# agsiddhant/PBML_Mantle_Convection

Measured on AMD Instinct MI355X. Metric: training samples/sec (2-D 506x506 Stokes fields), higher is better.
Workload: dtype f16+bf16; 1 GPU; CFG-3: symmetric U-Net (levels 5, c_h 16, k 5, repeats 3, reflect) + L1 data loss + divergence + Stokes momentum residual, 506x506, per-GPU batch 32, Adam, HIP-graph replay; global_batch=32, parallelism=dp1

## Files before the change

### include/mantle_hip.h

```cpp
#ifndef MANTLE_HIP_H
#define MANTLE_HIP_H

#include <stddef.h>
#include <stdint.h>

#ifdef __cplusplus
extern "C" {
#endif

#define MC_OK 0
#define MC_EINVAL (-1)
#define MC_EUNSUPPORTED (-2)
#define MC_EWORKSPACE (-3)

enum { MC_F32 = 0, MC_BF16 = 1, MC_MIX16 = 2 };
enum { MC_PAD_ZEROS = 0, MC_PAD_REPLICATE = 1, MC_PAD_REFLECT = 2 };
enum { MC_ACT_NONE = 0, MC_ACT_GELU = 1, MC_ACT_RELU = 2, MC_ACT_SILU = 3, MC_ACT_TANH = 4,
       MC_ACT_SELU = 5, MC_ACT_ELU = 6 };
enum { MC_POST_NONE = 0,
       MC_POST_ACT = 1,
       MC_POST_GN_ACT = 2   };
enum { MC_GSRC_NONE = 0,
       MC_GSRC_PLAIN = 1,
       MC_GSRC_PADFOLD = 2,
       MC_GSRC_PADFOLD_POOL = 3,
       MC_GSRC_PLAIN_POOL = 4   };

typedef struct {
  int32_t n;
  int32_t h, w;
  int32_t c_in0;
  int32_t c_in1;
  int32_t c_out;
  int32_t k;
  int32_t pad;
  int32_t pad_mode;
  int32_t dtype;
  int32_t sym_h;
  int32_t c_out_split;
  int32_t out_f32;
  int32_t sym_v;
  int32_t sym_hv;
} mc_conv_desc;

typedef struct {
  const void* ptr;
  int32_t kind;
  int32_t pad;
  int32_t pad_mode;
  int32_t pool;
  int32_t hs, ws;
  int32_t c8_total;
  int32_t cb_off;
} mc_grad_src;

typedef struct {
  const float* coef0;
  const float* coef1;
  int32_t act0, act1;
} mc_conv_prologue;

typedef struct {
  const void* y;
  const float* coef;
  int32_t act;
  int32_t pad;
  int32_t pad_mode;
  int32_t hs, ws;
  float* partials;
  int32_t part_stride;
  int32_t y_f16;
} mc_conv_epilogue;

int mc_version(void);
const char* mc_strerror(int code);

int mc_pack_nchw(const float* x, int32_t n, int32_t c, int32_t src_c, int32_t h, int32_t w, int32_t pad_w,
                 int32_t pad_mode, const float* chan_scale, int32_t dtype, void* out, void* stream);
int mc_unpack_nchw(const void* x, int32_t n, int32_t c, int32_t h, int32_t w, int32_t crop_w,
                   const float* mean_nc, int32_t dtype, float* out, void* stream);
int mc_pack_grad_nchw(const float* g, int32_t n, int32_t c, int32_t h, int32_t w, int32_t crop_w,
                      const float* mean_nc, int32_t dtype, void* out, void* stream);
int mc_sum_hw(const float* x, int32_t nc, int32_t hw, float scale, float* out, void* stream);

size_t mc_packed_weight_bytes(const mc_conv_desc* d, int32_t dgrad);
int mc_pack_weights(const mc_conv_desc* d, const float* w_unique, int32_t dgrad, void* packed,
                    void* stream);
const char* mc_conv_kernel_name(const mc_conv_desc* d);
int32_t mc_conv_tiles(const mc_conv_desc* d);
int mc_conv2d(const mc_conv_desc* d, const void* x0, const void* x1, const void* packed_w,
              const float* bias, void* y0, void* y1, float* stat_partials, void* stream);
int mc_conv2d_fused(const mc_conv_desc* d, const void* x0, const void* x1, const mc_conv_prologue* pro,
                    const void* packed_w, const float* bias, void* y0, void* y1, float* stat_partials,
                    const mc_conv_epilogue* epi, void* stream);
size_t mc_wgrad_partial_bytes(const mc_conv_desc* d);
size_t mc_conv_bank_read_extent(const mc_conv_desc* d);
int mc_conv2d_wgrad(const mc_conv_desc* d, const void* x0, const void* x1, const void* dy,
                    void* partials, void* stream);
int mc_conv2d_wgrad_finalize(const mc_conv_desc* d, const void* partials, float* dw_unique,
                             float* dbias, void* stream);
int mc_conv2d_wgrad_fused(const mc_conv_desc* d, const void* x0, const void* x1, const mc_conv_prologue* pro,
                          const void* dy, void* partials, void* stream);
int mc_pack_weights_batched(const mc_conv_desc* descs, const float* const* w_unique, const int32_t* dgrad,
                            void* const* packed, int32_t n, void* stream);
int mc_conv2d_wgrad_finalize_batched(const mc_conv_desc* descs, const void* const* partials, float* const* dw_unique,
                                     float* const* dbias, int32_t n, void* stream);

int mc_fold_padded(void* buf, int32_t n, int32_t c, int32_t hs, int32_t ws, int32_t pad, int32_t pad_mode,
                   int32_t dtype, void* stream);
int mc_fold_padded2(void* buf0, int32_t c0, void* buf1, int32_t c1, int32_t n, int32_t hs, int32_t ws, int32_t pad, int32_t pad_mode,
                    int32_t dtype, void* stream);
int32_t mc_fold_blocks(int32_t hs, int32_t ws, int32_t pad, int32_t pad_mode);
int mc_fold_padded_dz(void* buf, int32_t n, int32_t c, int32_t hs, int32_t ws, int32_t pad, int32_t pad_mode,
                      int32_t dtype, const void* y, const float* coef, int32_t act, float* partials,
                      int32_t part_stride_blocks, int32_t part_first_block, void* stream);

int mc_gn_partials(const void* y, int32_t n, int32_t c, int32_t h, int32_t w, int32_t dtype, int32_t tiles, float* part,
                   void* stream);
int mc_gn_finalize(const float* stat_partials, int32_t n, int32_t tiles, int32_t c, int32_t groups,
                   int32_t hw, float eps, float* stats_ng2, float* chan_mean, void* stream);
int mc_gn_finalize_coef(const float* stat_partials, int32_t n, int32_t tiles, int32_t c, int32_t groups, int32_t hw,
                        float eps, const float* gamma, const float* beta, float* stats_ng2, float* coef4, void* stream);

int mc_gn_act_fwd(const void* y, int32_t n, int32_t c, int32_t h, int32_t w, int32_t groups,
                  const float* stats_ng2, const float* gamma, const float* beta, int32_t post,
                  int32_t act, int32_t pool, int32_t dtype, void* a, void* pooled, void* stream);
int mc_gn_act_fwd_small(const void* y, const float* stat_partials, int32_t tiles, int32_t n, int32_t c, int32_t h, int32_t w,
                        int32_t groups, float eps, const float* gamma, const float* beta, int32_t act, int32_t pool,
                        int32_t dtype, float* stats_ng2, void* a, void* pooled, void* stream);
int32_t mc_gn_bwd_blocks(int32_t h, int32_t w);
int mc_gn_act_bwd_reduce(const void* y, int32_t n, int32_t c, int32_t h, int32_t w, int32_t groups,
                         const float* stats_ng2, const float* gamma, const float* beta, int32_t post,
                         int32_t act, int32_t dtype, const mc_grad_src* g0, const mc_grad_src* g1,
                         float* partials, void* stream);
int mc_gn_act_bwd_finalize(const float* partials, int32_t n, int32_t blocks, int32_t c, int32_t groups,
                           int32_t hw, const float* gamma, float* m12_ng2, float* dgamma, float* dbeta,
                           void* stream);
int mc_gn_act_bwd_finalize_n(const float* partials, int32_t n, int32_t blocks, int32_t c, int32_t groups, int32_t hw,
                             const float* gamma, float* m12_ng2, float* chan_sums, void* stream);
int mc_gn_act_bwd_apply(const void* y, int32_t n, int32_t c, int32_t h, int32_t w, int32_t groups,
                        const float* stats_ng2, const float* m12_ng2, const float* gamma,
                        const float* beta, int32_t post, int32_t act, int32_t dtype,
                        const mc_grad_src* g0, const mc_grad_src* g1, void* dy, void* stream);
int mc_gn_act_bwd_small(const void* y, int32_t n, int32_t c, int32_t h, int32_t w, int32_t groups, const float* stats_ng2,
                        const float* gamma, const float* beta, int32_t act, int32_t dtype, const mc_grad_src* g0,
                        const mc_grad_src* g1, void* dy, float* chan_sums, void* stream);
int mc_gn_param_grads_batched(const float* const* chan_sums, const int32_t* n, const int32_t* c, float* const* dgamma,
                              float* const* dbeta, int32_t jobs, void* stream);
int mc_gn_bwd_apply_dz(const mc_grad_src* dz, const void* y, int32_t n, int32_t c, int32_t h, int32_t w, int32_t groups,
                       const float* coef, const float* m12_ng2, int32_t dtype, void* dy, void* stream);
int mc_concat_cb8(const void* const* srcs, const int32_t* src_c, int32_t n_src, int32_t n, int32_t h, int32_t w,
                  int32_t dtype, void* out, void* stream);
int mc_cat_grad_gather(const mc_grad_src* g, int32_t c_total, int32_t c_off, int32_t c, int32_t n, int32_t h, int32_t w,
                       int32_t dtype, void* out, void* stream);
int mc_gsrc_sum(const mc_grad_src* g0, const mc_grad_src* g1, int32_t n, int32_t c, int32_t h, int32_t w,
                int32_t dtype, void* out, void* stream);

int mc_rect_copy(const void* src, int32_t hs, int32_t ws, int32_t sy, int32_t sx, void* dst, int32_t hd, int32_t wd,
                 int32_t dy, int32_t dx, int32_t rh, int32_t rw, int32_t n, int32_t c, int32_t accumulate, int32_t dtype,
                 void* stream);

typedef struct {
  int32_t n;
  int32_t h, w;
  int32_t c_in, c_out;
  int32_t k;
  int32_t bc_x, bc_y;
  int32_t dtype;
  int32_t sym_h;
} mc_learned_desc;

int32_t mc_learned_validate(const mc_learned_desc* d);
size_t mc_learned_bank_bytes(const mc_learned_desc* d, int32_t dgrad);
size_t mc_learned_wgrad_workspace_bytes(const mc_learned_desc* d);
int mc_learned_pack_banks_batched(const mc_learned_desc* descs, const float* const* w_unique, void* const* fwd_banks,
                                  void* const* dgrad_banks, int32_t n, void* stream);
int mc_learned_frame_fwd(const mc_learned_desc* d, const void* x, const void* fwd_bank, const float* bias, void* y,
                         void* stream);
int mc_learned_frame_dgrad(const mc_learned_desc* d, const void* dy, const void* dgrad_bank, void* dx, void* stream);
int mc_learned_frame_wgrad(const mc_learned_desc* d, const void* x, const void* dy, void* workspace,
                           float* const* dw_unique, float* dbias, void* stream);

int mc_avgpool_fwd(const void* x, int32_t n, int32_t c, int32_t h, int32_t w, int32_t f, int32_t dtype,
                   void* out, void* stream);
int mc_bicubic_fwd(const void* x, int32_t n, int32_t c, int32_t hi, int32_t wi, int32_t ho, int32_t wo,
// ... 95 lines not shown
```

### pbml_mantle_convection_amd/_lib.py

```python
import ctypes as C
import os

import torch

_HERE = os.path.dirname(os.path.abspath(__file__))
LIB_PATH = os.environ.get("MANTLE_LIB", os.path.join(_HERE, "libmantle_hip.so"))

MC_F32, MC_BF16, MC_MIX16 = 0, 1, 2
PAD_MODES = {"zeros": 0, "constant": 0, "replicate": 1, "reflect": 2}
ACTS = {"none": 0, "gelu": 1, "relu": 2, "silu": 3, "tanh": 4, "selu": 5, "elu": 6}
POST_NONE, POST_ACT, POST_GN_ACT = 0, 1, 2
GSRC_NONE, GSRC_PLAIN, GSRC_PADFOLD, GSRC_PADFOLD_POOL, GSRC_PLAIN_POOL = 0, 1, 2, 3, 4
LOSS_SLOTS = 16
LOSS_TYPES = {"mae": 0, "mass": 1, "curl": 2}


class ConvDesc(C.Structure):
    _fields_ = [(n, C.c_int32) for n in ("n", "h", "w", "c_in0", "c_in1", "c_out", "k", "pad", "pad_mode",
                                          "dtype", "sym_h", "c_out_split", "out_f32", "sym_v", "sym_hv")]


class LearnedDesc(C.Structure):
    _fields_ = [(n, C.c_int32) for n in ("n", "h", "w", "c_in", "c_out", "k", "bc_x", "bc_y", "dtype", "sym_h")]


LEARNED_FRAME_BANKS = ("conv_bottom_left", "conv_bottom", "conv_bottom_right", "conv_left", "conv_right", "conv_top_left",
                       "conv_top", "conv_top_right")


class GradSrc(C.Structure):
    _fields_ = [("ptr", C.c_void_p), ("kind", C.c_int32), ("pad", C.c_int32), ("pad_mode", C.c_int32),
                ("pool", C.c_int32), ("hs", C.c_int32), ("ws", C.c_int32), ("c8_total", C.c_int32), ("cb_off", C.c_int32)]


class ConvPrologue(C.Structure):
    _fields_ = [("coef0", C.c_void_p), ("coef1", C.c_void_p), ("act0", C.c_int32), ("act1", C.c_int32)]


class ConvEpilogue(C.Structure):
    _fields_ = [("y", C.c_void_p), ("coef", C.c_void_p), ("act", C.c_int32), ("pad", C.c_int32), ("pad_mode", C.c_int32),
                ("hs", C.c_int32), ("ws", C.c_int32), ("partials", C.c_void_p), ("part_stride", C.c_int32),
                ("y_f16", C.c_int32)]


class LossDesc(C.Structure):
    _fields_ = [("n", C.c_int32), ("h", C.c_int32), ("w", C.c_int32), ("p_pred", C.c_int32),
                ("loss_type", C.c_int32), ("loss_scale", C.c_int32), ("loss_derivative", C.c_int32),
                ("l2", C.c_int32), ("lambda_mom", C.c_float), ("inv_h", C.c_float), ("ra", C.c_float),
                ("t_grad", C.c_int32)]


_vp, _i32, _i64, _f32, _sz = C.c_void_p, C.c_int32, C.c_int64, C.c_float, C.c_size_t
_CD, _GS, _LD = C.POINTER(ConvDesc), C.POINTER(GradSrc), C.POINTER(LossDesc)
_CP, _CE = C.POINTER(ConvPrologue), C.POINTER(ConvEpilogue)
_LN = C.POINTER(LearnedDesc)

SIGNATURES = {
    "mc_version": (C.c_int, []),
    "mc_strerror": (C.c_char_p, [C.c_int]),
    "mc_pack_nchw": (C.c_int, [_vp, _i32, _i32, _i32, _i32, _i32, _i32, _i32, _vp, _i32, _vp, _vp]),
    "mc_unpack_nchw": (C.c_int, [_vp, _i32, _i32, _i32, _i32, _i32, _vp, _i32, _vp, _vp]),
    "mc_pack_grad_nchw": (C.c_int, [_vp, _i32, _i32, _i32, _i32, _i32, _vp, _i32, _vp, _vp]),
    "mc_sum_hw": (C.c_int, [_vp, _i32, _i32, _f32, _vp, _vp]),
    "mc_packed_weight_bytes": (_sz, [_CD, _i32]),
    "mc_conv_bank_read_extent": (_sz, [_CD]),
    "mc_pack_weights": (C.c_int, [_CD, _vp, _i32, _vp, _vp]),
    "mc_conv_tiles": (_i32, [_CD]),
    "mc_conv_kernel_name": (C.c_char_p, [_CD]),
    "mc_conv2d": (C.c_int, [_CD, _vp, _vp, _vp, _vp, _vp, _vp, _vp, _vp]),
    "mc_conv2d_fused": (C.c_int, [_CD, _vp, _vp, _CP, _vp, _vp, _vp, _vp, _vp, _CE, _vp]),
    "mc_conv2d_wgrad_fused": (C.c_int, [_CD, _vp, _vp, _CP, _vp, _vp, _vp]),
    "mc_gn_finalize_coef": (C.c_int, [_vp, _i32, _i32, _i32, _i32, _i32, _f32, _vp, _vp, _vp, _vp, _vp]),
    "mc_fold_blocks": (_i32, [_i32, _i32, _i32, _i32]),
    "mc_fold_padded_dz": (C.c_int, [_vp, _i32, _i32, _i32, _i32, _i32, _i32, _i32, _vp, _vp, _i32, _vp, _i32, _i32, _vp]),
    "mc_gn_bwd_apply_dz": (C.c_int, [_GS, _vp, _i32, _i32, _i32, _i32, _i32, _vp, _vp, _i32, _vp, _vp]),
    "mc_bicubic_fwd_act": (C.c_int, [_vp, _vp, _i32, _i32, _i32, _i32, _i32, _i32, _i32, _vp, _vp, _vp, _vp, _i32, _vp,
                                     _vp]),
    "mc_wgrad_partial_bytes": (_sz, [_CD]),
    "mc_conv2d_wgrad": (C.c_int, [_CD, _vp, _vp, _vp, _vp, _vp]),
    "mc_conv2d_wgrad_finalize": (C.c_int, [_CD, _vp, _vp, _vp, _vp]),
    "mc_pack_weights_batched": (C.c_int, [_CD, _vp, _vp, _vp, _i32, _vp]),
    "mc_conv2d_wgrad_finalize_batched": (C.c_int, [_CD, _vp, _vp, _vp, _i32, _vp]),
    "mc_fold_padded": (C.c_int, [_vp, _i32, _i32, _i32, _i32, _i32, _i32, _i32, _vp]),
    "mc_fold_padded2": (C.c_int, [_vp, _i32, _vp, _i32, _i32, _i32, _i32, _i32, _i32, _i32, _vp]),
    "mc_gn_partials": (C.c_int, [_vp, _i32, _i32, _i32, _i32, _i32, _i32, _vp, _vp]),
    "mc_gn_finalize": (C.c_int, [_vp, _i32, _i32, _i32, _i32, _i32, _f32, _vp, _vp, _vp]),
    "mc_gn_act_fwd": (C.c_int, [_vp, _i32, _i32, _i32, _i32, _i32, _vp, _vp, _vp, _i32, _i32, _i32, _i32, _vp,
                                _vp, _vp]),
    "mc_gn_bwd_blocks": (_i32, [_i32, _i32]),
    "mc_gn_act_bwd_reduce": (C.c_int, [_vp, _i32, _i32, _i32, _i32, _i32, _vp, _vp, _vp, _i32, _i32, _i32, _GS,
                                       _GS, _vp, _vp]),
    "mc_gn_act_bwd_finalize": (C.c_int, [_vp, _i32, _i32, _i32, _i32, _i32, _vp, _vp, _vp, _vp, _vp]),
    "mc_gn_act_bwd_finalize_n": (C.c_int, [_vp, _i32, _i32, _i32, _i32, _i32, _vp, _vp, _vp, _vp]),
    "mc_gn_act_bwd_apply": (C.c_int, [_vp, _i32, _i32, _i32, _i32, _i32, _vp, _vp, _vp, _vp, _i32, _i32, _i32,
                                      _GS, _GS, _vp, _vp]),
    "mc_gn_act_fwd_small": (C.c_int, [_vp, _vp, _i32, _i32, _i32, _i32, _i32, _i32, _f32, _vp, _vp, _i32, _i32, _i32, _vp, _vp, _vp,
                                      _vp]),
    "mc_gn_act_bwd_small": (C.c_int, [_vp, _i32, _i32, _i32, _i32, _i32, _vp, _vp, _vp, _i32, _i32, _GS, _GS, _vp, _vp, _vp]),
    "mc_gn_param_grads_batched": (C.c_int, [_vp, _vp, _vp, _vp, _vp, _i32, _vp]),
    "mc_avgpool_fwd": (C.c_int, [_vp, _i32, _i32, _i32, _i32, _i32, _i32, _vp, _vp]),
    "mc_rect_copy": (C.c_int, [_vp, _i32, _i32, _i32, _i32, _vp, _i32, _i32, _i32, _i32, _i32, _i32, _i32, _i32, _i32, _i32,
                               _vp]),
    "mc_learned_validate": (_i32, [_LN]),
    "mc_learned_bank_bytes": (_sz, [_LN, _i32]),
    "mc_learned_wgrad_workspace_bytes": (_sz, [_LN]),
    "mc_learned_pack_banks_batched": (C.c_int, [_LN, _vp, _vp, _vp, _i32, _vp]),
    "mc_learned_frame_fwd": (C.c_int, [_LN, _vp, _vp, _vp, _vp, _vp]),
    "mc_learned_frame_dgrad": (C.c_int, [_LN, _vp, _vp, _vp, _vp]),
    "mc_learned_frame_wgrad": (C.c_int, [_LN, _vp, _vp, _vp, _vp, _vp, _vp]),
    "mc_concat_cb8": (C.c_int, [_vp, _vp, _i32, _i32, _i32, _i32, _i32, _vp, _vp]),
    "mc_gsrc_sum": (C.c_int, [_GS, _GS, _i32, _i32, _i32, _i32, _i32, _vp, _vp]),
    "mc_cat_grad_gather": (C.c_int, [_GS, _i32, _i32, _i32, _i32, _i32, _i32, _i32, _vp, _vp]),
    "mc_bicubic_fwd": (C.c_int, [_vp, _i32, _i32, _i32, _i32, _i32, _i32, _vp, _vp, _vp, _vp, _i32, _vp, _vp]),
    "mc_bicubic_bwd": (C.c_int, [_GS, _i32, _i32, _i32, _i32, _i32, _i32, _vp, _vp, _vp, _vp, _vp, _vp, _i32,
                                 _vp, _vp]),
    "mc_bicubic_bwd_walk": (C.c_int, [_GS, _i32, _i32, _i32, _i32, _i32, _i32, _vp, _vp, _vp, _vp, _vp, _vp, _vp, _i32, _i32, _vp, _vp]),
    "mc_bicubic_bwd_taps": (C.c_int, [_GS, _i32, _i32, _i32, _i32, _i32, _i32, _vp, _vp, _vp, _vp, _vp, _vp, _i32, _i32, _i32,
                                      _vp, _vp]),
    "mc_bicubic_bwd_separable": (C.c_int, [_GS, _i32, _i32, _i32, _i32, _i32, _i32, _vp, _vp, _vp, _vp, _vp, _vp, _i32,
                                           _vp, _vp, _vp]),
    "mc_curl_head_fwd": (C.c_int, [_vp, _vp, _i32, _i32, _i32, _i64, _f32, _f32, _f32, _vp, _vp, _vp, _vp]),
    "mc_curl_head_bwd": (C.c_int, [_vp, _vp, _vp, _vp, _i32, _i32, _i32, _f32, _f32, _f32, _vp, _vp, _i64, _i64,
                                   _vp, _vp]),
    "mc_curl_valid_fwd": (C.c_int, [_vp, _i32, _i32, _i32, _i64, _f32, _vp, _vp, _vp]),
    "mc_curl_valid_bwd": (C.c_int, [_vp, _vp, _i32, _i32, _i32, _f32, _vp, _i64, _vp]),
    "mc_assemble_adtime_batch": (C.c_int, [_vp, _vp, _vp, _vp, _vp, _vp, _vp, _vp, _i32, _i32, _i32, _i32, _i32, _vp, _vp,
                                           _vp, _vp, _vp]),
    "mc_assemble_newad_batch": (C.c_int, [_vp, _vp, _vp, _vp, _vp, _vp, _vp, _vp, _i32, _i32, _i32, _i32, _i32, _vp, _vp, _vp, _vp, _vp]),
    "mc_ts_build_input": (C.c_int, [_vp, _vp, _vp, _vp, _vp, _vp, _i32, _i32, _i32, _vp, _vp]),
    "mc_ts_build_input_unet": (C.c_int, [_vp, _vp, _vp, _vp, _vp, _vp, _vp, _vp, _vp, _i32, _i32, _i32, _vp, _vp]),
    "mc_roll_forward_update": (C.c_int, [_vp, _i32, _vp, _vp, _vp, _i64, _vp, _i32, _i32, _i32, _i32, _vp]),
    "mc_ts_wall_bc": (C.c_int, [_vp, _i32, _i32, _i32, _vp, _vp]),
    "mc_adnet_step": (C.c_int, [_vp, _vp, _i64, _vp, _vp, _vp, _vp, _vp, _vp, _i32, _i32, _i32, _f32, _i32, _vp, _vp, _vp,
                                _vp]),
    "mc_loss_minmax": (C.c_int, [_vp, _i32, _i32, _i32, _i32, _vp, _vp]),
    "mc_loss_fwd_bwd": (C.c_int, [_LD, _vp, _vp, _vp, _vp, _i64, _i64, _vp, _vp, _vp, _vp, _vp, _vp, _vp, _vp]),
    "mc_loss_fused": (C.c_int, [_LD, _vp, _vp, _vp, _vp, _i64, _i64, _vp, _i32, _i32, _vp, _i32, _vp, _vp, _vp, _vp, _vp, _vp, _vp, _vp,
                                _vp, _vp, _i64, _i64, _vp, _vp]),
    "mc_loss_fused_blocks": (_i32, [_i32, _i32, _i32]),
    "mc_partial_sums_finalize": (C.c_int, [_vp, _i32, _i32, _i32, _f32, _vp, _vp]),
    "mc_momentum_residual": (C.c_int, [_LD, _vp, _vp, _vp, _vp, _i64, _i64, _vp, _vp, _vp, _vp, _vp, _vp, _vp, _vp]),
    "mc_momentum_adjoint": (C.c_int, [_LD, _vp, _i64, _i64, _vp, _vp, _vp, _vp, _vp, _vp, _vp, _vp, _vp, _vp]),
    "mc_loss_finalize": (C.c_int, [_LD, _vp, _vp, _vp]),
    "mc_adam_step_flat": (C.c_int, [_vp, _vp, _vp, _vp, _i64, _vp, _f32, _f32, _f32, _f32, _f32, _vp, _vp]),
}

VALUE_RETURNING = {"mc_version", "mc_strerror", "mc_conv_kernel_name", "mc_packed_weight_bytes", "mc_conv_bank_read_extent", "mc_conv_tiles",
                   "mc_wgrad_partial_bytes", "mc_gn_bwd_blocks",
                   "mc_learned_validate", "mc_learned_bank_bytes", "mc_learned_wgrad_workspace_bytes", "mc_fold_blocks", "mc_loss_fused_blocks"}

_lib = None


def load():
# ... 50 lines not shown
```

### pbml_mantle_convection_amd/build_ext.py

```python
import os
import subprocess
import sys

HERE = os.path.dirname(os.path.abspath(__file__))
CSRC = os.path.join(HERE, "csrc")
LIB = os.path.join(HERE, "libmantle_hip.so")
SOURCES = ["elementwise.hip", "conv_api.hip", "conv_f32.hip", "conv_bf16.hip", "conv_rr_bf16.hip", "conv_learned.hip", "loss.hip", "optim.hip"]
HEADERS = ["common.h", "conv_common.h", "conv_rr.h", os.path.join("..", "..", "include", "mantle_hip.h")]
FLAGS = ["-O3", "--offload-arch=gfx950", "-fPIC", "-std=c++17", "-Wall", "-Wno-unused-function",
         "-ffp-contract=off"]


EXTRA_FLAGS = {"conv_rr_bf16.hip": ["-fno-slp-vectorize"]}


def _stale(target, deps):
    if not os.path.exists(target):
        return True
    t = os.path.getmtime(target)
    return any(os.path.getmtime(d) > t for d in deps)


def build(force=False, verbose=True):
    hipcc = os.environ.get("HIPCC", "/opt/rocm/bin/hipcc")
    hdrs = [os.path.join(CSRC, h) for h in HEADERS]
    objdir = os.path.join(HERE, "build")
    os.makedirs(objdir, exist_ok=True)
    objs = []
    procs = []
    for src in SOURCES:
        s = os.path.join(CSRC, src)
        o = os.path.join(objdir, src.replace(".hip", ".o"))
        objs.append(o)
        if force or _stale(o, [s] + hdrs):
            cmd = [hipcc, *FLAGS, *EXTRA_FLAGS.get(src, []), "-c", s, "-o", o]
            if verbose:
                print(" ".join(cmd), flush=True)
            procs.append((src, subprocess.Popen(cmd)))
    for src, p in procs:
        if p.wait() != 0:
            raise RuntimeError(f"hipcc failed on {src}")
    if force or procs or _stale(LIB, objs):
        cmd = [hipcc, "--offload-arch=gfx950", "-shared", "-fPIC", *objs, "-o", LIB]
        if verbose:
            print(" ".join(cmd), flush=True)
        subprocess.check_call(cmd)
    return LIB


if __name__ == "__main__":
    build(force="--force" in sys.argv)
    print(LIB)
```

### pbml_mantle_convection_amd/csrc/common.h

```cpp
#pragma once
#include <hip/hip_runtime.h>
#include <stdint.h>
#include "../../include/mantle_hip.h"

typedef uint16_t bf16_t;

#define MC_CHECK_LAUNCH()                                 \
  do {                                                    \
    hipError_t e__ = hipGetLastError();                   \
    if (e__ != hipSuccess) return (int)e__;               \
  } while (0)

static inline int cdiv(int a, int b) { return (a + b - 1) / b; }

__device__ __forceinline__ float bf2f(bf16_t v) { return __uint_as_float(((uint32_t)v) << 16); }
__device__ __forceinline__ bf16_t f2bf(float f) {
  __bf16 b = (__bf16)f;
  return __builtin_bit_cast(bf16_t, b);
}
typedef float mc_f32x2 __attribute__((ext_vector_type(2)));
typedef __bf16 mc_bf16x2 __attribute__((ext_vector_type(2)));
__device__ __forceinline__ uint32_t pk_bf16(float a, float b) {
  return __builtin_bit_cast(uint32_t, __builtin_convertvector((mc_f32x2){a, b}, mc_bf16x2));
}
// ... 177 lines not shown
}
template <bool FAST>
__device__ __forceinline__ void act_bwd8(const float (&v)[8], const float (&sc)[8], const float (&sh)[8], int act, float (&o)[8]) {
  if (FAST && act == MC_ACT_GELU) {
#pragma unroll
    for (int j = 0; j < 8; j += 2) {
      f32x2 z = pk_fma((f32x2){v[j], v[j + 1]}, (f32x2){sc[j], sc[j + 1]}, (f32x2){sh[j], sh[j + 1]});
      f32x2 r = gelu_grad_poly2(z);
      o[j] = r.x; o[j + 1] = r.y;
    }
  } else {
#pragma unroll
    for (int j = 0; j < 8; ++j) o[j] = act_bwd(v[j] * sc[j] + sh[j], act);
  }
}
template <typename T> struct FastMath { static constexpr bool value = false; };
template <> struct FastMath<bf16_t> { static constexpr bool value = true; };
template <> struct FastMath<f16_t> { static constexpr bool value = true; };
__host__ __device__ inline bool mc_is16(int dtype) { return dtype == MC_BF16 || dtype == MC_MIX16; }

__device__ __forceinline__ void load_coef8(const float* __restrict__ coef4, int n, int CP, int cb, float (&sc)[8], float (&sh)[8]) {
  if (coef4) {
    const float4* p = reinterpret_cast<const float4*>(coef4) + (size_t)n * CP + cb * 8;
#pragma unroll
    for (int j = 0; j < 8; ++j) { const float4 v = p[j]; sc[j] = v.x; sh[j] = v.y; }
  } else {
#pragma unroll
    for (int j = 0; j < 8; ++j) { sc[j] = 1.f; sh[j] = 0.f; }
  }
}
__device__ __forceinline__ uint4 xform_bf16x8(uint4 a, const float (&sc)[8], const float (&sh)[8], int act) {
  float v[8];
  v[0] = __uint_as_float(a.x << 16); v[1] = __uint_as_float(a.x & 0xffff0000u);
  v[2] = __uint_as_float(a.y << 16); v[3] = __uint_as_float(a.y & 0xffff0000u);
  v[4] = __uint_as_float(a.z << 16); v[5] = __uint_as_float(a.z & 0xffff0000u);
  v[6] = __uint_as_float(a.w << 16); v[7] = __uint_as_float(a.w & 0xffff0000u);
  act_fwd8<true>(v, sc, sh, act, v);
  uint4 o;
  o.x = pk_bf16(v[0], v[1]);
  o.y = pk_bf16(v[2], v[3]);
  o.z = pk_bf16(v[4], v[5]);
  o.w = pk_bf16(v[6], v[7]);
  return o;
}

__device__ __forceinline__ uint4 xform_f16x8(uint4 a, const float (&sc)[8], const float (&sh)[8], int act) {
  float v[8];
  V8<f16_t>::ld(reinterpret_cast<const f16_t*>(&a), v);
  act_fwd8<true>(v, sc, sh, act, v);
  return make_uint4(pk_f16(v[0], v[1]), pk_f16(v[2], v[3]), pk_f16(v[4], v[5]), pk_f16(v[6], v[7]));
}
__device__ __forceinline__ uint4 f16x8_to_bf16x8(uint4 a) {
  const mc_f32x2 x = unpk_f16(a.x), y = unpk_f16(a.y), z = unpk_f16(a.z), w = unpk_f16(a.w);
  return make_uint4(pk_bf16(x.x, x.y), pk_bf16(y.x, y.y), pk_bf16(z.x, z.y), pk_bf16(w.x, w.y));
}

__device__ __forceinline__ float wave_sum(float v) {
#pragma unroll
  for (int o = 32; o > 0; o >>= 1) v += __shfl_xor(v, o, 64);
  return v;
}
__device__ __forceinline__ double wave_sum_d(double v) {
#pragma unroll
  for (int o = 32; o > 0; o >>= 1) v += __shfl_xor(v, o, 64);
  return v;
}

__device__ __forceinline__ float wave_sum16(const float (&s)[16], int lane, int& idx) {
  float t[8], u[4], v[2], w;
  const bool b5 = lane & 32, b4 = lane & 16, b3 = lane & 8, b2 = lane & 4;
#pragma unroll
  for (int k = 0; k < 8; ++k) t[k] = (b5 ? s[8 + k] : s[k]) + __shfl_xor(b5 ? s[k] : s[8 + k], 32, 64);
#pragma unroll
  for (int k = 0; k < 4; ++k) u[k] = (b4 ? t[4 + k] : t[k]) + __shfl_xor(b4 ? t[k] : t[4 + k], 16, 64);
#pragma unroll
  for (int k = 0; k < 2; ++k) v[k] = (b3 ? u[2 + k] : u[k]) + __shfl_xor(b3 ? u[k] : u[2 + k], 8, 64);
  w = (b2 ? v[1] : v[0]) + __shfl_xor(b2 ? v[0] : v[1], 4, 64);
  w += __shfl_xor(w, 2, 64);
  w += __shfl_xor(w, 1, 64);
  idx = (b5 ? 8 : 0) + (b4 ? 4 : 0) + (b3 ? 2 : 0) + (b2 ? 1 : 0);
  return w;
}

__device__ __forceinline__ int fold_candidates(int i, int n, int p, int mode, int (&out)[6]) {
  int cnt = 0;
  out[cnt++] = i + p;
  if (mode == MC_PAD_REFLECT) {
    if (i >= 1 && i <= p) out[cnt++] = p - i;
    int j = 2 * (n - 1) - i;
    if (j >= n && j < n + p) out[cnt++] = j + p;
  } else if (mode == MC_PAD_REPLICATE) {
    if (i == 0) for (int q = 0; q < p && cnt < 6; ++q) out[cnt++] = q;
    if (i == n - 1) for (int q = 0; q < p && cnt < 6; ++q) out[cnt++] = n + p + q;
  }
  return cnt;
}

template <typename T, int KIND = -1>
__device__ __forceinline__ void grad_fetch_add(const mc_grad_src& g, int n, int cb, int y, int x, int C8,
                                               float (&acc)[8]) {
  const int kind = KIND >= 0 ? KIND : g.kind;
  if (kind == MC_GSRC_NONE || (KIND < 0 && g.ptr == nullptr)) return;
  const T* base = reinterpret_cast<const T*>(g.ptr);
  if (KIND < 0 && g.c8_total > 0) { C8 = g.c8_total; cb += g.cb_off; }
  float v[8];
  if (kind == MC_GSRC_PLAIN) {
    V8<T>::ld(base + cb8_index(n, cb, y, x, C8, g.hs, g.ws), v);
#pragma unroll
    for (int j = 0; j < 8; ++j) acc[j] += v[j];
    return;
  }
  float scale = 1.0f;
  int yy = y, xx = x;
  if (kind == MC_GSRC_PADFOLD_POOL || kind == MC_GSRC_PLAIN_POOL) {
    if (g.pool == 2) { yy = y >> 1; xx = x >> 1; } else { yy = y / g.pool; xx = x / g.pool; }
    if (yy >= g.hs || xx >= g.ws) return;
    scale = 1.0f / (float)(g.pool * g.pool);
  }
  const int pad = kind == MC_GSRC_PLAIN_POOL ? 0 : g.pad;
  V8<T>::ld(base + cb8_index(n, cb, yy + pad, xx + pad, C8, g.hs + 2 * pad, g.ws + 2 * pad), v);
#pragma unroll
  for (int j = 0; j < 8; ++j) acc[j] += scale * v[j];
}
```

### pbml_mantle_convection_amd/csrc/conv_api.hip

```cpp
#include "conv_rr.h"

int mc_conv2d_f32(const ConvGeom& g, const void* x0, const void* x1, const void* bank, const float* bias, void* y0,
                  void* y1, float* part, const ConvFuse& fz, int fuse, hipStream_t s);
int mc_wgrad_f32(const ConvGeom& g, const void* x0, const void* x1, const void* dy, void* part, const ConvFuse& fz, int fuse,
                 hipStream_t s);
int mc_bf16_tile(const mc_conv_desc* d, int* th, int* tw);
size_t mc_bf16_bank_bytes(const ConvGeom& g, int dgrad);
int mc_conv2d_bf16(const ConvGeom& g, const void* x0, const void* x1, const void* bank, const float* bias, void* y0,
                   void* y1, float* part, const ConvFuse& fz, int fuse, hipStream_t s);
int mc_wgrad_bf16(const ConvGeom& g, const void* x0, const void* x1, const void* dy, void* part, const ConvFuse& fz, int fuse,
                  hipStream_t s);
const char* mc_bf16_kernel_name(const ConvGeom& g);
void mc_bf16_bank_dims(const ConvGeom& g, int dgrad, int& chunks, int& steps, int& ntiles);
bool mc_rr_applies(int dtype, int cout, int wo, bool full_pad);
size_t mc_rr_bank_bytes(const ConvGeom& g, int dgrad);
int mc_conv2d_rr(const ConvGeom& g, const void* x0, const void* x1, const void* bank, const float* bias, void* y0, void* y1,
                 float* part, const ConvFuse& fz, int fuse, hipStream_t s);
const char* mc_rr_kernel_name(const ConvGeom& g, int fuse);

namespace {

bool rr_desc(const mc_conv_desc* d) {
  return mc_rr_applies(d->dtype, d->c_out, d->w + 2 * d->pad - d->k + 1, d->pad == d->k - 1);
}

int geom_for(const mc_conv_desc* d, ConvGeom& g) {
  if (!d) return MC_EINVAL;
  int th = 16, tw = 16;
  if (mc_is16(d->dtype)) {
    if (rr_desc(d)) { th = RR_R; tw = RR_TW; }
    else {
      int rc = mc_bf16_tile(d, &th, &tw);
      if (rc) return rc;
    }
  } else if (d->dtype != MC_F32) {
    return MC_EUNSUPPORTED;
  }
  return conv_geom(d, th, tw, g);
}
int stat_slots(const mc_conv_desc* d, const ConvGeom& g) { return rr_desc(d) ? g.tiles * RR_STRIPS : g.tiles; }

struct PkJob {
  int K, Cout, CBin, CB0, Cin0, Cin1, Cin, U, nh, nv, nq, CBout, CinP, CoutP;
  int dgrad, steps, ntiles, bf16, f16, rr, first_block;
  unsigned total;
  const float* w;
  void* out;
};
constexpr int PK_MAX = 24;
struct PkTable { int n; PkJob j[PK_MAX]; };

__global__ void k_pack_batched(PkTable t) {
  int ji = 0;
#pragma unroll 1
  for (int k = 1; k < t.n; ++k) if ((int)blockIdx.x >= t.j[k].first_block) ji = k;
  const PkJob& job = t.j[ji];
  const int nblk = (ji + 1 < t.n ? t.j[ji + 1].first_block : (int)gridDim.x) - job.first_block;
  for (size_t i = (size_t)(blockIdx.x - job.first_block) * blockDim.x + threadIdx.x; i < job.total; i += (size_t)nblk * blockDim.x) {
    if (job.rr || job.bf16) {
      const float v = job.rr ? rr_pack_value(job, job.w, i, job.dgrad, job.ntiles)
                             : pack_value_bf16(job, job.w, i, job.dgrad, job.steps, job.ntiles);
      reinterpret_cast<bf16_t*>(job.out)[i] = job.f16 ? __builtin_bit_cast(bf16_t, (_Float16)v) : f2bf(v);
    } else {
      reinterpret_cast<float*>(job.out)[i] = pack_value_f32(job, job.w, i, job.dgrad);
    }
  }
}

struct WfJob {
  int K, U, nh, nv, nq, Cin, Cin0, CB0, CinP, CoutP, Cout, G, first_block;
  const float* part;
  float* dw;
  float* db;
};
constexpr int WF_MAX = 32;
struct WfTable { int n; WfJob j[WF_MAX]; };

constexpr int WF_WAVES = 16;
__device__ __forceinline__ void wgrad_finalize_block(const WfJob& g, int lblock) {
  const int K = g.K, KK = K * K;
  const int nch = wg_chunks(g.CinP);
  const size_t slab = wg_slab_floats(g.CoutP, g.CinP, KK);
  const size_t nW = (size_t)KK * nch * g.U * 16;
  const size_t total = nW + g.Cout;
  const int e = threadIdx.x & 63, w = threadIdx.x >> 6, NWV = (int)blockDim.x >> 6;
  const size_t i = (size_t)lblock * 64 + e;
  __shared__ float red[WF_WAVES][64];
  float s = 0.f;
  long dst = -1;
  if (i < total) {
    size_t o1, ox[3] = {0, 0, 0};
    int nx = 0;
    bool live = true;
    if (i < nW) {
// ... 105 lines not shown
  if (geom_for(d, g)) return "unsupported";
  if (rr_desc(d)) return mc_rr_kernel_name(g, 0);
  if (mc_is16(g.dtype)) return mc_bf16_kernel_name(g);
  return g.K == 5 ? "k_conv_direct_f32<5>" : "k_conv_direct_f32<3>";
}

int32_t mc_conv_tiles(const mc_conv_desc* d) {
  ConvGeom g;
  if (geom_for(d, g)) return -1;
  return stat_slots(d, g);
}

static bool act_ok(int a) { return a >= MC_ACT_NONE && a <= MC_ACT_ELU; }

static int fill_prologue(const mc_conv_prologue* pro, ConvFuse& fz, int& rc) {
  rc = MC_OK;
  if (!pro) return 0;
  if (!act_ok(pro->act0) || !act_ok(pro->act1)) { rc = MC_EINVAL; return 0; }
  fz.coef0 = pro->coef0; fz.coef1 = pro->coef1; fz.act0 = pro->act0; fz.act1 = pro->act1;
  return (pro->coef0 || pro->coef1 || pro->act0 != MC_ACT_NONE || pro->act1 != MC_ACT_NONE) ? 1 : 0;
}

int mc_conv2d_fused(const mc_conv_desc* d, const void* x0, const void* x1, const mc_conv_prologue* pro,
                    const void* packed_w, const float* bias, void* y0, void* y1, float* stat_partials,
                    const mc_conv_epilogue* epi, void* stream) {
  ConvGeom g;
  int rc = geom_for(d, g);
  if (rc) return rc;
  if (!x0 || !packed_w || !y0 || (g.Cin1 > 0 && !x1) || (g.split8 > 0 && !y1)) return MC_EINVAL;
  ConvFuse fz = conv_fuse_none();
  int fuse = fill_prologue(pro, fz, rc);
  if (rc) return rc;
  if (epi) {
    if (fuse) return MC_EUNSUPPORTED;
    if (!epi->y || !epi->partials || !act_ok(epi->act) || epi->pad < 0 || epi->hs <= 0 || epi->ws <= 0) return MC_EINVAL;
    if (epi->pad_mode < MC_PAD_ZEROS || epi->pad_mode > MC_PAD_REFLECT) return MC_EINVAL;
    if (g.split8 > 0 || stat_partials || g.out_f32) return MC_EUNSUPPORTED;
    if (g.Ho != epi->hs + 2 * epi->pad || g.Wo != epi->ws + 2 * epi->pad) return MC_EINVAL;
    fz.ey = epi->y; fz.ecoef = epi->coef; fz.epart = epi->partials; fz.eact = epi->act; fz.epad = epi->pad;
    fz.ezero = epi->pad_mode == MC_PAD_ZEROS || epi->pad == 0; fz.ehs = epi->hs; fz.ews = epi->ws;
    if (epi->y_f16 && g.dtype != MC_BF16) return MC_EINVAL;
    fz.ey16 = epi->y_f16 ? 1 : 0;
    if (epi->part_stride < stat_slots(d, g)) return MC_EINVAL;
    fz.estride = epi->part_stride;
    fuse = 2;
  }
  if (rr_desc(d)) return mc_conv2d_rr(g, x0, x1, packed_w, bias, y0, y1, stat_partials, fz, fuse, (hipStream_t)stream);
  if (mc_is16(g.dtype)) return mc_conv2d_bf16(g, x0, x1, packed_w, bias, y0, y1, stat_partials, fz, fuse, (hipStream_t)stream);
  return mc_conv2d_f32(g, x0, x1, packed_w, bias, y0, y1, stat_partials, fz, fuse, (hipStream_t)stream);
}

int mc_conv2d(const mc_conv_desc* d, const void* x0, const void* x1, const void* packed_w, const float* bias, void* y0,
              void* y1, float* stat_partials, void* stream) {
  return mc_conv2d_fused(d, x0, x1, nullptr, packed_w, bias, y0, y1, stat_partials, nullptr, stream);
}

size_t mc_conv_bank_read_extent(const mc_conv_desc* d) {
  ConvGeom g;
  if (geom_for(d, g)) return 0;
  const int KK = g.K * g.K;
  if (rr_desc(d)) {
    const size_t nfrag = g.K == 5 ? RR<5>::NFRAG : RR<3>::NFRAG;
    const size_t chunks = (g.CBin + 1) / 2, groups = (g.Cout + 15) / 16;
    return (((chunks - 1) * groups + (groups - 1)) * nfrag * 64 + (nfrag * 64 - 1)) * 16 + 16;
  }
  if (mc_is16(g.dtype)) {
    int chunks, steps, ntiles;
    mc_bf16_bank_dims(g, 0, chunks, steps, ntiles);
    const size_t last = ((size_t)(chunks - 1) * steps + (steps - 1)) * ntiles + (ntiles - 1);
    return (last * 64 + 63) * 16 + 16;
  }
  const int ncog = (g.CoutP + 15) / 16, co0 = 16 * (ncog - 1);
  const int comax = g.CoutP - 1 - co0;
  const size_t last = (((size_t)(g.CBin - 1) * KK + (KK - 1)) * 8 + 7) * g.CoutP + co0 + (comax >= 15 ? 15 : comax);
  return (last + 1) * sizeof(float);
}

size_t mc_wgrad_partial_bytes(const mc_conv_desc* d) {
  ConvGeom g;
  if (geom_for(d, g)) return 0;
  return (size_t)g.wgrad_G * wg_slab_floats(g.CoutP, g.CinP, g.K * g.K) * sizeof(float);
}

int mc_conv2d_wgrad_fused(const mc_conv_desc* d, const void* x0, const void* x1, const mc_conv_prologue* pro,
                          const void* dy, void* partials, void* stream) {
  ConvGeom g;
  int rc = geom_for(d, g);
  if (rc) return rc;
  if (!x0 || !dy || !partials || (g.Cin1 > 0 && !x1)) return MC_EINVAL;
  ConvFuse fz = conv_fuse_none();
  const int fuse = fill_prologue(pro, fz, rc);
  if (rc) return rc;
  if (mc_is16(g.dtype)) return mc_wgrad_bf16(g, x0, x1, dy, partials, fz, fuse, (hipStream_t)stream);
  return mc_wgrad_f32(g, x0, x1, dy, partials, fz, fuse, (hipStream_t)stream);
}

int mc_conv2d_wgrad(const mc_conv_desc* d, const void* x0, const void* x1, const void* dy, void* partials,
                    void* stream) {
  return mc_conv2d_wgrad_fused(d, x0, x1, nullptr, dy, partials, stream);
}

int mc_conv2d_wgrad_finalize_batched(const mc_conv_desc* descs, const void* const* partials, float* const* dw,
                                     float* const* db, int32_t n, void* stream) {
  if (!descs || !partials || !dw || !db || n <= 0) return MC_EINVAL;
  for (int pass = 0; pass < 2; ++pass) {
    WfTable t;
    t.n = 0;
    int blocks = 0;
    auto flush = [&]() {
      if (t.n == 0) return;
      hipLaunchKernelGGL(k_wgrad_finalize, dim3(blocks), dim3(pass == 0 ? 64 * WF_WAVES : 256), 0, (hipStream_t)stream, t);
      t.n = 0; blocks = 0;
    };
    for (int k = 0; k < n; ++k) {
      WfJob j;
      int b = 0;
      int rc = wf_fill(&descs[k], partials[k], dw[k], db[k], j, b);
      if (rc) return rc;
      if ((j.G >= 128) != (pass == 0)) continue;
      j.first_block = blocks;
      t.j[t.n++] = j;
      blocks += b;
      if (t.n == WF_MAX) flush();
    }
    flush();
    MC_CHECK_LAUNCH();
  }
  return MC_OK;
}

int mc_conv2d_wgrad_finalize(const mc_conv_desc* d, const void* partials, float* dw_unique, float* dbias,
                             void* stream) {
  return mc_conv2d_wgrad_finalize_batched(d, &partials, &dw_unique, &dbias, 1, stream);
}

int mc_pack_weights_batched(const mc_conv_desc* descs, const float* const* w_unique, const int32_t* dgrad,
                            void* const* packed, int32_t n, void* stream) {
  if (!descs || !w_unique || !dgrad || !packed || n <= 0) return MC_EINVAL;
  for (int base = 0; base < n; base += PK_MAX) {
    PkTable t;
    t.n = n - base < PK_MAX ? n - base : PK_MAX;
    int blocks = 0;
    for (int k = 0; k < t.n; ++k) {
      ConvGeom g;
      int rc = geom_for(&descs[base + k], g);
      if (rc) return rc;
      if (!w_unique[base + k] || !packed[base + k]) return MC_EINVAL;
      PkJob& j = t.j[k];
      j.K = g.K; j.Cout = g.Cout; j.CBin = g.CBin; j.CB0 = g.CB0; j.Cin0 = g.Cin0; j.Cin1 = g.Cin1; j.Cin = g.Cin; j.U = g.U;
      j.nh = g.nh; j.nv = g.nv; j.nq = g.nq;
      j.CBout = g.CBout; j.CinP = g.CinP; j.CoutP = g.CoutP; j.dgrad = dgrad[base + k]; j.bf16 = mc_is16(g.dtype);
      j.f16 = (g.dtype == MC_MIX16 && !j.dgrad) ? 1 : 0;
      j.rr = bank_is_rr(g, j.dgrad);
      size_t total;
      if (j.rr) {
        j.steps = 0;
        j.ntiles = ((j.dgrad ? g.CinP : g.Cout) + 15) / 16;
        total = mc_rr_bank_bytes(g, j.dgrad) / 2;
      } else if (j.bf16) {
        int chunks;
        mc_bf16_bank_dims(g, j.dgrad, chunks, j.steps, j.ntiles);
        total = (size_t)chunks * j.steps * j.ntiles * 64 * 8;
      } else {
        j.steps = 0; j.ntiles = 0;
        total = (size_t)(j.dgrad ? g.CBout : g.CBin) * g.K * g.K * 8 * (j.dgrad ? g.CinP : g.CoutP);
      }
      j.total = (unsigned)total;
      j.w = w_unique[base + k];
      j.out = packed[base + k];
      j.first_block = blocks;
      int b = (int)((total + 256 * 8 - 1) / (256 * 8));
      blocks += b < 1 ? 1 : b;
    }
    hipLaunchKernelGGL(k_pack_batched, dim3(blocks), dim3(256), 0, (hipStream_t)stream, t);
    MC_CHECK_LAUNCH();
  }
  return MC_OK;
// ... 12 lines not shown
```

### pbml_mantle_convection_amd/csrc/conv_bf16.hip

```cpp
#include "conv_common.h"
#include <type_traits>

using bf16x8 = __attribute__((ext_vector_type(8))) short;
using f16x8 = __attribute__((ext_vector_type(8))) _Float16;
using f32x4 = __attribute__((ext_vector_type(4))) float;
typedef unsigned int v4u __attribute__((ext_vector_type(4)));

namespace {

constexpr int CHUNK_CB = 2;

template <int K> struct KSteps { static constexpr int pairs = K * K * CHUNK_CB; static constexpr int steps = (pairs + 3) / 4; };

struct Bf16Cfg { int th, tw, nt, mt; };

__host__ __device__ inline int pick_nt(int n_tiles) { return (n_tiles % 4 == 0) ? 4 : ((n_tiles % 2 == 0) ? 2 : 1); }


template <bool H16> __device__ __forceinline__ f32x4 mfma16(bf16x8 a, bf16x8 b, f32x4 c) {
  if constexpr (H16) return __builtin_amdgcn_mfma_f32_16x16x32_f16(__builtin_bit_cast(f16x8, a), __builtin_bit_cast(f16x8, b), c, 0, 0, 0);
  else return __builtin_amdgcn_mfma_f32_16x16x32_bf16(a, b, c, 0, 0, 0);
}

template <int K, int TH, int TW, int NT, int MT, bool OUT_F32 = false, int FUSE = 0, bool H16 = false, int WN = 1>
__global__ __launch_bounds__(64 * (TH * (TW / 16) / MT) * WN, 2) void k_conv_mfma_bf16(
    ConvGeom g, const bf16_t* __restrict__ x0, const bf16_t* __restrict__ x1, const bf16_t* __restrict__ bank,
    const float* __restrict__ bias, bf16_t* __restrict__ y0, bf16_t* __restrict__ y1, float* __restrict__ part,
    int n_groups, ConvFuse fz) {
  constexpr int TIH = TH + K - 1, TIW = TW + K - 1;
  constexpr int PLANE = (TIH * TIW + 15) / 16 * 16;
  constexpr int STEPS = KSteps<K>::steps;
  constexpr int MTILES_X = TW / 16;
  constexpr int WAVES = TH * MTILES_X / MT * WN, NTHR = 64 * WAVES;
  constexpr int NTW = NT / WN;
  static_assert(TH * MTILES_X * WN == WAVES * MT && NTW * WN == NT && (WAVES == 4 || WAVES == 8), "tile / wave decomposition mismatch");
  constexpr int IN_SLOTS = CHUNK_CB * PLANE;
  constexpr bool WGLOBAL = NT > 1;
  constexpr int W_SLOTS = WGLOBAL ? 0 : STEPS * NT * 64;
  static_assert(!OUT_F32 || NT == 1, "f32 output is for the single-N-tile configuration");
  constexpr int IN_ELEMS = CHUNK_CB * TIH * TIW;
  constexpr int IN_ITERS = (IN_ELEMS + NTHR - 1) / NTHR;
  constexpr int W_ITERS = WGLOBAL ? 1 : (W_SLOTS + NTHR - 1) / NTHR;
  __shared__ uint4 lds[IN_SLOTS + (WGLOBAL ? 1 : W_SLOTS)];
  __shared__ float red[WAVES][NT * 16 * 2];
  uint4* in_s = lds;
  uint4* w_s = lds + IN_SLOTS;

  const int grp = blockIdx.y;
  const int bid = xcd_remap(blockIdx.x, gridDim.x);
  const int lane = threadIdx.x & 63, wave = __builtin_amdgcn_readfirstlane(threadIdx.x >> 6);
  const int m = lane & 15, gq = lane >> 4;
  const int ntile0 = grp * NT;
  const int wm = wave / WN, nt_w0 = (wave % WN) * NTW;
  const int ntiles_total = gridDim.y * NT;
  const int chunks = (g.CBin + CHUNK_CB - 1) / CHUNK_CB;
  const int items = g.N * g.tiles;
  const int my_items = (items - bid + (int)gridDim.x - 1) / (int)gridDim.x;
  const int total_stages = my_items * chunks;

  constexpr int PER_CB = (TIH * TIW + NTHR - 1) / NTHR;
  static_assert(IN_ITERS <= CHUNK_CB * PER_CB, "");
  v4u rin[CHUNK_CB][PER_CB];
  float psc[CHUNK_CB][8], psh[CHUNK_CB][8];
  int pact[CHUNK_CB] = {-1, -1};
  unsigned okm = 0xffffffffu;
  int s_rc[PER_CB];
  unsigned s_off[PER_CB];
  int s_lds[PER_CB];
#pragma unroll
  for (int it = 0; it < PER_CB; ++it) {
    int i = threadIdx.x + it * NTHR;
    bool live = i < TIH * TIW;
    if (!live) i = TIH * TIW - 1;
    int r = i / TIW, c = i - r * TIW;
    s_rc[it] = (live ? 0 : (1 << 31)) | (r << 15) | c;
    s_off[it] = (unsigned)(r * g.W + c) * 16u;
    s_lds[it] = live ? r * TIW + c : -1;
  }
  auto prefetch = [&](int t) {
    const int jitem = t / chunks, ck = t - jitem * chunks;
    const int wi = bid + jitem * (int)gridDim.x;
    const int n = wi / g.tiles, tile = wi - n * g.tiles;
    const int ty0 = (tile / g.tiles_x) * TH, tx0 = (tile % g.tiles_x) * TW;
// ... 243 lines not shown
          const size_t off = (size_t)(i / MTILES_X) * row_bytes + (size_t)(i % MTILES_X) * 16 * 8 * 2;
          float yf[4];
          if constexpr (H16) {
            const f32x2 ya = unpk_f16(yv[i].x), yb = unpk_f16(yv[i].y);
            yf[0] = ya.x; yf[1] = ya.y; yf[2] = yb.x; yf[3] = yb.y;
          } else {
            yf[0] = __uint_as_float(yv[i].x << 16); yf[1] = __uint_as_float(yv[i].x & 0xffff0000u);
            yf[2] = __uint_as_float(yv[i].y << 16); yf[3] = __uint_as_float(yv[i].y & 0xffff0000u);
          }
          float o[4];
#pragma unroll
          for (int h = 0; h < 2; ++h) {
            const f32x2 yy = (f32x2){yf[2 * h], yf[2 * h + 1]};
            const f32x2 z = pk_fma(yy, (f32x2){csc[2 * h], csc[2 * h + 1]}, (f32x2){csh[2 * h], csh[2 * h + 1]});
            f32x2 gp;
            if (fz.eact == MC_ACT_GELU) gp = gelu_grad_poly2(z);
            else gp = (f32x2){act_bwd(z.x, fz.eact), act_bwd(z.y, fz.eact)};
            const f32x2 da = (f32x2){acc[i][tt][2 * h], acc[i][tt][2 * h + 1]};
            const f32x2 dz = da * gp;
            const f32x2 yh = (yy - (f32x2){cme[2 * h], cme[2 * h + 1]}) * (f32x2){crs[2 * h], crs[2 * h + 1]};
            if (fin[i]) { s1[tt][h] += dz; s2[tt][h] = pk_fma(dz, yh, s2[tt][h]); }
            o[2 * h] = fin[i] ? dz.x : da.x; o[2 * h + 1] = fin[i] ? dz.y : da.y;
          }
          if (inb && cobok[tt]) {
            uint2 pk;
            pk.x = (uint32_t)f2bf(o[0]) | ((uint32_t)f2bf(o[1]) << 16);
            pk.y = (uint32_t)f2bf(o[2]) | ((uint32_t)f2bf(o[3]) << 16);
            *reinterpret_cast<uint2*>(dst0[tt] + off) = pk;
          }
        }
      }
    };
    if constexpr (FUSE == 2) emit_dz();
    else { if (ty0 + TH <= g.Ho && tx0 + TW <= g.Wo) emit(std::true_type{}); else emit(std::false_type{}); }
    STAMP(5);
    if (FUSE == 2) part = fz.epart;
    if (part) {
#pragma unroll
      for (int tt = 0; tt < NTW; ++tt) {
        float q8[8] = {s1[tt][0].x, s2[tt][0].x, s1[tt][0].y, s2[tt][0].y, s1[tt][1].x, s2[tt][1].x, s1[tt][1].y, s2[tt][1].y};
        const bool b3 = m & 8, b2 = m & 4, b1 = m & 2;
        float q4[4], q2[2], q1;
#pragma unroll
        for (int k = 0; k < 4; ++k) q4[k] = (b3 ? q8[4 + k] : q8[k]) + __shfl_xor(b3 ? q8[k] : q8[4 + k], 8, 64);
#pragma unroll
        for (int k = 0; k < 2; ++k) q2[k] = (b2 ? q4[2 + k] : q4[k]) + __shfl_xor(b2 ? q4[k] : q4[2 + k], 4, 64);
        q1 = (b1 ? q2[1] : q2[0]) + __shfl_xor(b1 ? q2[0] : q2[1], 2, 64);
        q1 += __shfl_xor(q1, 1, 64);
        if ((m & 1) == 0) red[wave][((nt_w0 + tt) * 16 + gq * 4) * 2 + (m >> 1)] = q1;
      }
      __syncthreads();
      if (threadIdx.x < NT * 32) {
        int co = ntile0 * 16 + (threadIdx.x >> 1);
        if (co < g.CoutP) {
          float r = 0.f;
#pragma unroll
          for (int wv = 0; wv < WAVES / WN; ++wv) r += red[wv * WN + (int)(threadIdx.x >> 5) / NTW][threadIdx.x];
          part[(((size_t)n * (FUSE == 2 ? fz.estride : g.tiles) + tile) * g.CoutP + co) * 2 + (threadIdx.x & 1)] = r;
        }
      }
    }
    STAMP(6);
  }
#ifdef MC_EXP_STAMPS
  if (blockIdx.x == 777 && blockIdx.y == 0 && threadIdx.x == 0)
    printf("stamps tiles %d: wait1 %lld commit %lld wait2 %lld pfetch %lld kloop %lld epi %lld stats %lld\n", my_items, st_acc[0], st_acc[1], st_acc[2], st_acc[3], st_acc[4], st_acc[5], st_acc[6]);
#endif
}

typedef short v4s __attribute__((ext_vector_type(4)));
typedef __attribute__((address_space(3))) v4s lds_v4s;

__device__ __forceinline__ bf16x8 tr_frag(const short* base_lo) {
  v4s lo = __builtin_amdgcn_ds_read_tr16_b64_v4i16((lds_v4s*)base_lo);
  v4s hi = __builtin_amdgcn_ds_read_tr16_b64_v4i16((lds_v4s*)(base_lo + 32));
  return (bf16x8){lo[0], lo[1], lo[2], lo[3], hi[0], hi[1], hi[2], hi[3]};
}

constexpr int WTH = 16, WTW = 32;

template <int K, int NTW, bool PRO = false, bool XH = false>
__global__ __launch_bounds__(256, NTW == 1 ? 3 : 2) void k_wgrad_mfma_bf16(ConvGeom g, const bf16_t* __restrict__ x0,
                                                            const bf16_t* __restrict__ x1, const bf16_t* __restrict__ dy,
                                                            float* __restrict__ part, int tiles_x, int tiles, ConvFuse fz) {
  constexpr int NS = 4;
  constexpr int TPW = (K * K + NS) / NS;
  constexpr int KK = K * K;
  constexpr int TIH = WTH + K - 1, TIW = WTW + K - 1;
  constexpr int XRS = (TIW + 11) / 16 * 16 + 4;
  constexpr int DRS = WTW + 4;
  constexpr int XPS = (TIH * XRS + 15) / 16 * 16 + 8;
  constexpr int DPS = WTH * DRS + 8;
  static_assert(XRS >= TIW && XRS >= 3 * 8 + 12 && XRS % 16 == 4 && DRS % 16 == 4 && XPS % 16 == 8 && DPS % 16 == 8,
                "register-shift LDS layout");
  constexpr int NACC = TPW * NTW;
  constexpr int X_ITERS = (TIH * TIW + 255) / 256;
  constexpr int D_ELEMS = NTW * 2 * WTH * WTW, D_ITERS = D_ELEMS / 256;
  static_assert(D_ELEMS % 256 == 0, "dy tile must divide evenly over the threads");
  __shared__ uint4 smem[2 * XPS + NTW * 2 * DPS];
  uint4* const xs = smem;
  uint4* const ds = smem + 2 * XPS;
  const int chunk = blockIdx.y, cog = blockIdx.z;
  const int bid = xcd_remap(blockIdx.x, gridDim.x);
  const int lane = threadIdx.x & 63, tg = __builtin_amdgcn_readfirstlane(threadIdx.x >> 6);
  const int q = (lane & 15) >> 2, p = lane & 3, gq = lane >> 4;
  const int lane_x = ((p >> 1) * XPS + gq * XRS + q) * 8 + (p & 1) * 4;
  const int lane_d = ((p >> 1) * DPS + gq * DRS + q) * 8 + (p & 1) * 4;
  const short* xs_s = reinterpret_cast<const short*>(xs);
  const short* ds_s = reinterpret_cast<const short*>(ds);
  const bool do_bias = tg == NS - 1 && chunk == 0;
  const bf16x8 ones = (bf16x8){0x3F80, 0x3F80, 0x3F80, 0x3F80, 0x3F80, 0x3F80, 0x3F80, 0x3F80};
  const ptrdiff_t x1_delta = x1 ? reinterpret_cast<const char*>(x1) - reinterpret_cast<const char*>(x0) : (ptrdiff_t)0;

  int x_rc[X_ITERS];
  unsigned x_off[X_ITERS];
#pragma unroll
  for (int it = 0; it < X_ITERS; ++it) {
    int i = threadIdx.x + it * 256;
    bool live = i < TIH * TIW;
    if (!live) i = TIH * TIW - 1;
    int r = i / TIW, c = i - r * TIW;
    x_rc[it] = (live ? 0 : (1 << 31)) | (r << 15) | c;
    x_off[it] = (unsigned)(r * g.W + c) * 16u;
  }
  static_assert(WTW == 32 && WTH == 16, "dy staging decode");
  const int d_r0 = threadIdx.x >> 5, d_c0 = threadIdx.x & 31;
  const unsigned d_off0 = (unsigned)(d_r0 * g.Wo + d_c0) * 16u;
  const int d_lds0 = d_r0 * DRS + d_c0;
  const bool co_full = (cog * NTW + NTW) * 2 <= g.CBout;
  const char* xbase[2];
  bool xok[2];
  int xC8[2];
#pragma unroll
  for (int cb = 0; cb < 2; ++cb) {
    int gcb = chunk * 2 + cb;
    xok[cb] = gcb < g.CBin;
    int gcc = min(gcb, g.CBin - 1);
    bool second = gcc >= g.CB0;
    xC8[cb] = second ? g.CB1 : g.CB0;
    xbase[cb] = reinterpret_cast<const char*>(x0) + (second ? x1_delta : (ptrdiff_t)0) +
                cb8_index(0, second ? gcc - g.CB0 : gcc, 0, 0, xC8[cb], g.H, g.W) * sizeof(bf16_t);
  }

  uint4 rx[2][X_ITERS], rd[D_ITERS];
  float psc[2][8], psh[2][8];
  int pact[2] = {-1, -1};
  unsigned okm = 0xffffffffu;
  auto prefetch = [&](int wi_fwd) __attribute__((always_inline)) {
    const int wi = wi_fwd;
    const int n = wi / tiles, tile = wi - n * tiles;
    const int ty0 = (tile / tiles_x) * WTH, tx0 = (tile % tiles_x) * WTW;
    const bool interior = (ty0 - g.pad >= 0) && (ty0 - g.pad + TIH <= g.H) && (tx0 - g.pad >= 0) && (tx0 - g.pad + TIW <= g.W);
    const char* bpn[2] = {xbase[0] + (size_t)n * xC8[0] * g.H * g.W * 16, xbase[1] + (size_t)n * xC8[1] * g.H * g.W * 16};
    if constexpr (PRO) {
#pragma unroll
      for (int cb = 0; cb < 2; ++cb) {
        const int gcb = min(chunk * 2 + cb, g.CBin - 1);
        const bool second = gcb >= g.CB0;
        const float* ct = second ? fz.coef1 : fz.coef0;
        const int a = second ? fz.act1 : fz.act0;
        pact[cb] = (xok[cb] && (ct != nullptr || a != MC_ACT_NONE)) ? a : -1;
        if (pact[cb] >= 0) load_coef8(ct, n, xC8[cb] * 8, second ? gcb - g.CB0 : gcb, psc[cb], psh[cb]);
      }
      okm = 0xffffffffu;
    }
    if (interior) {
      const size_t org = (size_t)((ty0 - g.pad) * g.W + (tx0 - g.pad)) * 16;
#pragma unroll
      for (int cb = 0; cb < 2; ++cb)
#pragma unroll
        for (int it = 0; it < X_ITERS; ++it) {
          uint4 v = *reinterpret_cast<const uint4*>(bpn[cb] + org + x_off[it]);
          rx[cb][it] = xok[cb] ? v : make_uint4(0, 0, 0, 0);
        }
    } else {
#pragma unroll
      for (int it = 0; it < X_ITERS; ++it) {
        int r = (x_rc[it] >> 15) & 0x7fff, c = x_rc[it] & 0x7fff;
        bool oky, okx;
        int sy = pad_map_sel(ty0 + r - g.pad, g.H, g.pad_mode, oky);
        int sx = pad_map_sel(tx0 + c - g.pad, g.W, g.pad_mode, okx);
        const bool ok = oky && okx;
// ... 150 lines not shown
}

}

int mc_bf16_tile(const mc_conv_desc* d, int* th, int* tw) {
  Bf16Cfg c = cfg_for(d->c_out, d->k, d->h + 2 * d->pad - d->k + 1);
  *th = c.th; *tw = c.tw;
  return MC_OK;
}

void mc_bf16_bank_dims(const ConvGeom& g, int dgrad, int& chunks, int& steps, int& ntiles) {
  int cb_in = dgrad ? g.CBout : g.CBin;
  int c_out = dgrad ? g.CinP : g.Cout;
  chunks = (cb_in + CHUNK_CB - 1) / CHUNK_CB;
  steps = g.K == 5 ? KSteps<5>::steps : KSteps<3>::steps;
  int nt_total = (c_out + 15) / 16;
  int nt = pick_nt(nt_total);
  ntiles = (nt_total + nt - 1) / nt * nt;
}

size_t mc_bf16_bank_bytes(const ConvGeom& g, int dgrad) {
  int chunks, steps, ntiles;
  mc_bf16_bank_dims(g, dgrad, chunks, steps, ntiles);
  return (size_t)chunks * steps * ntiles * 64 * 16;
}

const char* mc_bf16_kernel_name(const ConvGeom& g) {
  Bf16Cfg c = cfg_for(g.Cout, g.K, g.Ho);
  if (g.out_f32) return g.K == 5 ? "k_conv_mfma_bf16<5,16,32,1,8,true>" : "k_conv_mfma_bf16<3,16,32,1,8,true>";
  if (g.K == 5 && c.th == 24) return "k_conv_mfma_bf16<5,24,16,4,6,false>";
  if (g.K == 5 && c.th == 12) return c.nt == 2 ? "k_conv_mfma_bf16<5,12,16,2,3,false>" : "k_conv_mfma_bf16<5,12,16,4,6,false,2x2>";
  if (g.K == 5 && c.th == 8) return c.nt == 2 ? "k_conv_mfma_bf16<5,8,16,2,2,false>" : "k_conv_mfma_bf16<5,8,16,4,4,false,2x2>";
  if (g.K == 5) return c.nt == 1 ? "k_conv_mfma_bf16<5,16,32,1,8,false>" : (c.nt == 2 ? "k_conv_mfma_bf16<5,16,16,2,4,false>" : "k_conv_mfma_bf16<5,16,16,4,8,false,2x2>");
  return c.nt == 1 ? "k_conv_mfma_bf16<3,16,32,1,8,false>" : (c.nt == 2 ? "k_conv_mfma_bf16<3,16,16,2,4,false>" : "k_conv_mfma_bf16<3,16,16,4,8,false,2x2>");
}

int mc_conv2d_bf16(const ConvGeom& g_in, const void* x0, const void* x1, const void* bank, const float* bias, void* y0,
                   void* y1, float* part, const ConvFuse& fz, int fuse, hipStream_t s) {
  const ConvGeom& g = g_in;
  Bf16Cfg c = cfg_for(g.Cout, g.K, g.Ho);
  int nt_total = (g.Cout + 15) / 16;
  int groups = (nt_total + c.nt - 1) / c.nt;
  int items = g.tiles * g.N;
  static int cap_total = getenv("MC_CONV_CAP") ? atoi(getenv("MC_CONV_CAP")) : 4096;
  int cap = cap_total / groups > 0 ? cap_total / groups : 1;
  int bx = items < cap ? items : cap;
  dim3 grid(bx, groups, 1);
  if (fuse == 2 && g.out_f32) return MC_EUNSUPPORTED;
  const bool h16 = fuse == 2 ? fz.ey16 != 0 : g.dtype == MC_MIX16;
#define LAUNCH_H(K, TH, TW, NT, MT, F32, FU, H, WN)                                                                    \
  hipLaunchKernelGGL((k_conv_mfma_bf16<K, TH, TW, NT, MT, F32, FU, H, WN>), grid, dim3(64 * (TH * (TW / 16) / (MT)) * (WN)), 0, s, g, \
                     (const bf16_t*)x0, (const bf16_t*)x1, (const bf16_t*)bank, bias, (bf16_t*)y0, (bf16_t*)y1, part,  \
                     groups, fz)
#define LAUNCH_F(K, TH, TW, NT, MT, F32, FU, WN)                                                                       \
  do { if (h16) LAUNCH_H(K, TH, TW, NT, MT, F32, FU, true, WN); else LAUNCH_H(K, TH, TW, NT, MT, F32, FU, false, WN); } while (0)
#define LAUNCH_W(K, TH, TW, NT, MT, F32, WN)                                                                           \
  do { if (fuse == 0) LAUNCH_F(K, TH, TW, NT, MT, F32, 0, WN); else if (fuse == 1) LAUNCH_F(K, TH, TW, NT, MT, F32, 1, WN);   \
       else LAUNCH_F(K, TH, TW, NT, MT, false, 2, WN); } while (0)
#define LAUNCH(K, TH, TW, NT, MT, F32) LAUNCH_W(K, TH, TW, NT, MT, F32, 1)
#define LAUNCH4(K, TH, TW, MT) LAUNCH_W(K, TH, TW, 4, 2 * (MT), false, 2)
  if (g.out_f32) {
    if (g.K == 5) LAUNCH(5, 16, 32, 1, NT1_MT, true); else if (g.K == 3) LAUNCH(3, 16, 32, 1, NT1_MT, true); else return MC_EUNSUPPORTED;
  } else if (g.K == 5) {
    if (c.nt == 1) LAUNCH(5, 16, 32, 1, NT1_MT, false);
    else if (c.th == 24) LAUNCH_W(5, 24, 16, 4, 6, false, 1);
    else if (c.th == 12) { if (c.nt == 2) LAUNCH(5, 12, 16, 2, 3, false); else LAUNCH4(5, 12, 16, 3); }
    else if (c.th == 8) { if (c.nt == 2) LAUNCH(5, 8, 16, 2, 2, false); else LAUNCH4(5, 8, 16, 2); }
    else if (c.nt == 2) LAUNCH(5, 16, 16, 2, 4, false); else LAUNCH4(5, 16, 16, 4);
  } else if (g.K == 3) {
    if (c.nt == 1) LAUNCH(3, 16, 32, 1, NT1_MT, false); else if (c.nt == 2) LAUNCH(3, 16, 16, 2, 4, false); else LAUNCH4(3, 16, 16, 4);
  } else {
    return MC_EUNSUPPORTED;
  }
#undef LAUNCH4
#undef LAUNCH_W
#undef LAUNCH
#undef LAUNCH_F
#undef LAUNCH_H
  MC_CHECK_LAUNCH();
  return MC_OK;
}

int mc_wgrad_bf16(const ConvGeom& g_in, const void* x0, const void* x1, const void* dy, void* part, const ConvFuse& fz,
                  int fuse, hipStream_t s) {
  const ConvGeom& g = g_in;
  const int tiles_x = (g.Wo + WTW - 1) / WTW, tiles_y = (g.Ho + WTH - 1) / WTH;
  const int tiles = tiles_x * tiles_y;
  const int ntiles = (g.Cout + 15) / 16;
  const int ntw = pick_nt(ntiles) >= 2 ? 2 : 1;
  dim3 grid(g.wgrad_G, (g.CBin + 1) / 2, (ntiles + ntw - 1) / ntw);
  const bool xh = g.dtype == MC_MIX16;
#define WLAUNCH_X(K, NTW, PRO, XH)                                                                                     \
  hipLaunchKernelGGL((k_wgrad_mfma_bf16<K, NTW, PRO, XH>), grid, dim3(256), 0, s, g, (const bf16_t*)x0, (const bf16_t*)x1, \
                     (const bf16_t*)dy, (float*)part, tiles_x, tiles, fz)
#define WLAUNCH_P(K, NTW, PRO) do { if (xh) WLAUNCH_X(K, NTW, PRO, true); else WLAUNCH_X(K, NTW, PRO, false); } while (0)
#define WLAUNCH(K, NTW) do { if (fuse) WLAUNCH_P(K, NTW, true); else WLAUNCH_P(K, NTW, false); } while (0)
  if (g.K == 5) { if (ntw == 1) WLAUNCH(5, 1); else WLAUNCH(5, 2); }
  else if (g.K == 3) { if (ntw == 1) WLAUNCH(3, 1); else WLAUNCH(3, 2); }
  else return MC_EUNSUPPORTED;
#undef WLAUNCH
#undef WLAUNCH_P
#undef WLAUNCH_X
  MC_CHECK_LAUNCH();
  return MC_OK;
}
```

### pbml_mantle_convection_amd/csrc/elementwise.hip

```cpp
#include "common.h"

namespace {

__device__ __forceinline__ void split_index(size_t i, bool small, int Wd, int H, int C8, int& xo, int& y, int& cb, int& n) {
  if (small) {
    unsigned r = (unsigned)i;
    xo = (int)(r % (unsigned)Wd); r /= (unsigned)Wd;
    y = (int)(r % (unsigned)H); r /= (unsigned)H;
    cb = (int)(r % (unsigned)C8);
    n = (int)(r / (unsigned)C8);
  } else {
    xo = (int)(i % Wd);
    size_t r = i / Wd;
    y = (int)(r % H); r /= H;
    cb = (int)(r % C8);
    n = (int)(r / C8);
  }
}

template <typename T>
__global__ void k_pack_nchw(const float* __restrict__ x, int N, int C, int SC, int H, int W, int pad_w, int mode,
                            const float* __restrict__ cs, T* __restrict__ out) {
  const int Wp = W + 2 * pad_w, C8 = (C + 7) / 8;
  size_t total = (size_t)N * C8 * H * Wp;
  for (size_t i = blockIdx.x * (size_t)blockDim.x + threadIdx.x; i < total; i += (size_t)gridDim.x * blockDim.x) {
    int xo, y, cb, n;
    split_index(i, total <= 0xffffffffull, Wp, H, C8, xo, y, cb, n);
    int xs = pad_map(xo - pad_w, W, mode);
    float v[8];
#pragma unroll
    for (int j = 0; j < 8; ++j) {
      int c = cb * 8 + j;
      v[j] = (c < C && xs >= 0) ? x[(((size_t)n * SC + c) * H + y) * W + xs] * (cs ? cs[c] : 1.f) : 0.f;
    }
    V8<T>::st(out + i * 8, v);
  }
}

template <typename T>
__global__ void k_unpack_nchw(const T* __restrict__ x, int N, int C, int H, int W, int crop,
                              const float* __restrict__ mean_nc, float* __restrict__ out) {
  const int Wo = W - 2 * crop, C8 = (C + 7) / 8;
  size_t total = (size_t)N * C8 * H * Wo;
  for (size_t i = blockIdx.x * (size_t)blockDim.x + threadIdx.x; i < total; i += (size_t)gridDim.x * blockDim.x) {
    int xo, y, cb, n;
    split_index(i, total <= 0xffffffffull, Wo, H, C8, xo, y, cb, n);
    float v[8];
    V8<T>::ld(x + cb8_index(n, cb, y, xo + crop, C8, H, W), v);
#pragma unroll
    for (int j = 0; j < 8; ++j) {
      int c = cb * 8 + j;
      if (c < C) {
        float m = mean_nc ? mean_nc[n * C + c] : 0.f;
        out[(((size_t)n * C + c) * H + y) * Wo + xo] = v[j] - m;
      }
    }
  }
}

template <typename T>
__global__ void k_pack_grad_nchw(const float* __restrict__ g, int N, int C, int H, int W, int crop,
                                 const float* __restrict__ mean_nc, T* __restrict__ out) {
  const int Wi = W - 2 * crop, C8 = (C + 7) / 8;
  size_t total = (size_t)N * C8 * H * W;
  for (size_t i = blockIdx.x * (size_t)blockDim.x + threadIdx.x; i < total; i += (size_t)gridDim.x * blockDim.x) {
    int xo, y, cb, n;
    split_index(i, total <= 0xffffffffull, W, H, C8, xo, y, cb, n);
    int xi = xo - crop;
    float v[8];
#pragma unroll
    for (int j = 0; j < 8; ++j) {
      int c = cb * 8 + j;
      float val = 0.f;
      if (c < C) {
        if (xi >= 0 && xi < Wi) val = g[(((size_t)n * C + c) * H + y) * Wi + xi];
        if (mean_nc) val -= mean_nc[n * C + c];
      }
      v[j] = val;
    }
    V8<T>::st(out + i * 8, v);
  }
}

// ... 568 lines not shown
    grad_fetch_add<T, GKinds<GK>::k1>(g1, n, cb, yy, xx, a.C8, da);
    act_bwd8<FastMath<T>::value>(v, sc, sh, a.act, gz);
#pragma unroll
    for (int j = 0; j < 8; ++j) {
      const float dz = da[j] * gz[j];
      s[2 * j] += dz;
      s[2 * j + 1] += dz * (v[j] - mean[j]) * rstd[j];
    }
  }
  __shared__ float red[16][16];
  __shared__ float tot[16];
  {
    int idx;
    const float r = wave_sum16(s, threadIdx.x & 63, idx);
    if ((threadIdx.x & 3) == 0) red[threadIdx.x >> 6][idx] = r;
  }
  __syncthreads();
  if (threadIdx.x < 16) {
    float r = 0.f;
    const int nw = (int)blockDim.x >> 6;
    for (int w = 0; w < nw; ++w) r += red[w][threadIdx.x];
    tot[threadIdx.x] = r;
    const int c = cb * 8 + (threadIdx.x >> 1);
    if (c < CP) pc[((size_t)n * CP + c) * 2 + (threadIdx.x & 1)] = r;
  }
  __syncthreads();
  float cA[8], cB[8], cC[8];
  const float invM = 1.0f / ((float)a.cpg * (float)total);
#pragma unroll
  for (int j = 0; j < 8; ++j) {
    const int c = cb * 8 + j;
    float m1 = 0.f, m2 = 0.f;
    if (c < a.C) {
      const int j0 = (j / a.cpg) * a.cpg;
      for (int k = 0; k < a.cpg; ++k) {
        const float gk = a.gamma[cb * 8 + j0 + k];
        m1 += gk * tot[2 * (j0 + k)];
        m2 += gk * tot[2 * (j0 + k) + 1];
      }
      m1 *= invM; m2 *= invM;
    }
    cA[j] = rstd[j] * ga[j];
    cB[j] = -rstd[j] * rstd[j] * m2;
    cC[j] = -rstd[j] * m1;
  }
  for (int i = threadIdx.x; i < total; i += blockDim.x) {
    const int yy = i / a.W, xx = i - yy * a.W;
    float v[8], da[8] = {0, 0, 0, 0, 0, 0, 0, 0}, gz[8], o[8];
    const size_t idx = cb8_index(n, cb, yy, xx, a.C8, a.H, a.W);
    V8<TY>::ld(y + idx, v);
    grad_fetch_add<T, GKinds<GK>::k0>(g0, n, cb, yy, xx, a.C8, da);
    grad_fetch_add<T, GKinds<GK>::k1>(g1, n, cb, yy, xx, a.C8, da);
    act_bwd8<FastMath<T>::value>(v, sc, sh, a.act, gz);
#pragma unroll
    for (int j = 0; j < 8; j += 2) {
      const f32x2 dz = (f32x2){da[j], da[j + 1]} * (f32x2){gz[j], gz[j + 1]};
      const f32x2 t = (f32x2){v[j], v[j + 1]} - (f32x2){mean[j], mean[j + 1]};
      const f32x2 r = pk_fma((f32x2){cA[j], cA[j + 1]}, dz, pk_fma((f32x2){cB[j], cB[j + 1]}, t, (f32x2){cC[j], cC[j + 1]}));
      o[j] = r.x; o[j + 1] = r.y;
    }
    V8<T>::st(dy + idx, o);
  }
}

constexpr int GP_MAX = 32;
struct GpJob { const float* pc; float* dgamma; float* dbeta; int N, C, CP, first; };
struct GpTable { int n; GpJob j[GP_MAX]; };
__global__ void k_gn_param_grads(GpTable t) {
  const int i = blockIdx.x * blockDim.x + threadIdx.x;
  int ji = 0;
#pragma unroll 1
  for (int k = 1; k < t.n; ++k) if (i >= t.j[k].first) ji = k;
  const GpJob& j = t.j[ji];
  const int c = i - j.first;
  if (c >= j.C) return;
  float s1 = 0.f, s2 = 0.f;
  for (int n = 0; n < j.N; ++n) { s1 += j.pc[((size_t)n * j.CP + c) * 2]; s2 += j.pc[((size_t)n * j.CP + c) * 2 + 1]; }
  if (j.dgamma) j.dgamma[c] += s2;
  if (j.dbeta) j.dbeta[c] += s1;
}

template <typename T>
__global__ void k_fold_padded(T* __restrict__ buf, int C8, int H, int W, int p, int mode, int all, T* __restrict__ buf1, int C8a) {
  const int n = blockIdx.z;
  int cb = blockIdx.y;
  if (buf1 && cb >= C8a) { buf = buf1; cb -= C8a; C8 -= C8a; } else if (buf1) { C8 = C8a; }
  const int t = p + 1;
  const int band = all ? H * W : 2 * t * W;
  const int side = all ? 0 : (H - 2 * t) * 2 * t;
  const int Hp = H + 2 * p, Wp = W + 2 * p;
  for (int i = blockIdx.x * blockDim.x + threadIdx.x; i < band + side; i += gridDim.x * blockDim.x) {
    int yy, xx;
    if (all) {
      yy = i / W;
      xx = i - yy * W;
    } else if (i < band) {
      int r = i / W;
      xx = i - r * W;
      yy = r < t ? r : H - 2 * t + r;
    } else {
      int k = i - band;
      int r = k / (2 * t), c = k - r * 2 * t;
      yy = t + r;
      xx = c < t ? c : W - 2 * t + c;
    }
    int cy[6], cx[6];
    int ny = fold_candidates(yy, H, p, mode, cy), nx = fold_candidates(xx, W, p, mode, cx);
    if (ny == 1 && nx == 1) continue;
    float acc[8] = {0, 0, 0, 0, 0, 0, 0, 0};
    for (int a = 0; a < ny; ++a)
      for (int b = 0; b < nx; ++b) {
        float v[8];
        V8<T>::ld(buf + cb8_index(n, cb, cy[a], cx[b], C8, Hp, Wp), v);
#pragma unroll
        for (int j = 0; j < 8; ++j) acc[j] += v[j];
      }
    V8<T>::st(buf + cb8_index(n, cb, yy + p, xx + p, C8, Hp, Wp), acc);
  }
}

template <typename T, typename TY = T>
__global__ __launch_bounds__(256) void k_fold_padded_dz(T* __restrict__ buf, int C8, int H, int W, int p, int mode, int all,
                                                        const TY* __restrict__ y, const float* __restrict__ coef4, int act,
                                                        float* __restrict__ part, int stride, int first) {
  const int n = blockIdx.z, cb = blockIdx.y;
  const int t = p + 1;
  const int band = all ? H * W : 2 * t * W;
  const int side = all ? 0 : (H - 2 * t) * 2 * t;
  const int Hp = H + 2 * p, Wp = W + 2 * p, CP = C8 * 8;
  float sc[8], sh[8], me[8], rs[8];
#pragma unroll
  for (int j = 0; j < 8; ++j) {
    if (coef4) {
      const float4 c4 = reinterpret_cast<const float4*>(coef4)[(size_t)n * CP + cb * 8 + j];
      sc[j] = c4.x; sh[j] = c4.y; me[j] = c4.z; rs[j] = c4.w;
    } else { sc[j] = 1.f; sh[j] = 0.f; me[j] = 0.f; rs[j] = 0.f; }
  }
  float s[16];
#pragma unroll
  for (int j = 0; j < 16; ++j) s[j] = 0.f;
  const int i = blockIdx.x * blockDim.x + threadIdx.x;
  if (i < band + side) {
    int yy, xx;
    if (all) {
      yy = i / W;
      xx = i - yy * W;
    } else if (i < band) {
      int r = i / W;
      xx = i - r * W;
      yy = r < t ? r : H - 2 * t + r;
    } else {
      int k = i - band;
      int r = k / (2 * t), c = k - r * 2 * t;
      yy = t + r;
      xx = c < t ? c : W - 2 * t + c;
    }
    int cy[6], cx[6];
    const int ny = fold_candidates(yy, H, p, mode, cy), nx = fold_candidates(xx, W, p, mode, cx);
    float acc[8] = {0, 0, 0, 0, 0, 0, 0, 0};
    for (int a = 0; a < ny; ++a)
      for (int b = 0; b < nx; ++b) {
        float v[8];
        V8<T>::ld(buf + cb8_index(n, cb, cy[a], cx[b], C8, Hp, Wp), v);
#pragma unroll
        for (int j = 0; j < 8; ++j) acc[j] += v[j];
      }
    float yv[8], gz[8];
    V8<TY>::ld(y + cb8_index(n, cb, yy, xx, C8, H, W), yv);
    act_bwd8<FastMath<T>::value>(yv, sc, sh, act, gz);
#pragma unroll
    for (int j = 0; j < 8; ++j) {
      const float dz = acc[j] * gz[j];
      acc[j] = dz;
      s[2 * j] = dz;
      s[2 * j + 1] = dz * (yv[j] - me[j]) * rs[j];
    }
    V8<T>::st(buf + cb8_index(n, cb, yy + p, xx + p, C8, Hp, Wp), acc);
  }
  __shared__ float red[4][16];
  int idx;
  float r = wave_sum16(s, threadIdx.x & 63, idx);
  if ((threadIdx.x & 3) == 0) red[threadIdx.x >> 6][idx] = r;
  __syncthreads();
  if (threadIdx.x < 16) {
    float tot = red[0][threadIdx.x] + red[1][threadIdx.x] + red[2][threadIdx.x] + red[3][threadIdx.x];
    part[(((size_t)n * stride + first + blockIdx.x) * CP + cb * 8 + (threadIdx.x >> 1)) * 2 + (threadIdx.x & 1)] = tot;
  }
}

template <typename T, int GK, typename TY = T>
__global__ __launch_bounds__(256) void k_gn_bwd_apply_dz(mc_grad_src gs, const TY* __restrict__ y, int C, int C8, int H, int W,
                                                         int groups, const float* __restrict__ coef4,
                                                         const float* __restrict__ m12, T* __restrict__ dy, int rows_pb) {
  const int n = blockIdx.z, cb = blockIdx.y;
  float cA[8], cB[8], cC[8], me[8];
  const int cpg = C / groups;
#pragma unroll
  for (int j = 0; j < 8; ++j) {
    const int c = cb * 8 + j;
    cA[j] = (c < C) ? 1.f : 0.f; cB[j] = 0.f; cC[j] = 0.f; me[j] = 0.f;
    if (coef4 && c < C) {
      const float4 c4 = reinterpret_cast<const float4*>(coef4)[(size_t)n * C8 * 8 + c];
      const int g = c / cpg;
      const float m1 = m12[((size_t)n * groups + g) * 2], m2 = m12[((size_t)n * groups + g) * 2 + 1];
      cA[j] = c4.x;
      cB[j] = -c4.w * c4.w * m2;
      cC[j] = -c4.w * m1;
      me[j] = c4.z;
    }
  }
  const int y0 = blockIdx.x * rows_pb, nrows = min(rows_pb, H - y0);
  for (int i = threadIdx.x; i < nrows * W; i += blockDim.x) {
    const int ry = i / W, xx = i - ry * W, yy = y0 + ry;
    float v[8] = {0, 0, 0, 0, 0, 0, 0, 0}, dz[8] = {0, 0, 0, 0, 0, 0, 0, 0}, o[8];
    const size_t idx = cb8_index(n, cb, yy, xx, C8, H, W);
    if (coef4) V8<TY>::ld(y + idx, v);
    grad_fetch_add<T, GK>(gs, n, cb, yy, xx, C8, dz);
#pragma unroll
    for (int j = 0; j < 8; j += 2) {
      const f32x2 t = (f32x2){v[j], v[j + 1]} - (f32x2){me[j], me[j + 1]};
      const f32x2 r = pk_fma((f32x2){cA[j], cA[j + 1]}, (f32x2){dz[j], dz[j + 1]},
                             pk_fma((f32x2){cB[j], cB[j + 1]}, t, (f32x2){cC[j], cC[j + 1]}));
      o[j] = r.x; o[j + 1] = r.y;
    }
    V8<T>::st(dy + idx, o);
  }
}

constexpr int FOH = 16, FOW = 64, FWH = 12, FWW = 36;
template <typename T>
__device__ __forceinline__ void bicubic_direct(const T* __restrict__ x, int n, int cb, int C8, int Hi, int Wi, int yo, int xo,
                                               const int* __restrict__ iy, const float* __restrict__ wy,
                                               const int* __restrict__ ix, const float* __restrict__ wx, float (&acc)[8],
                                               const float* __restrict__ coef4, int act) {
  float sc[8], sh[8];
  if (act >= 0) load_coef8(coef4, n, C8 * 8, cb, sc, sh);
#pragma unroll
  for (int j = 0; j < 8; ++j) acc[j] = 0.f;
#pragma unroll
  for (int a = 0; a < 4; ++a) {
    int ys = iy[yo * 4 + a];
    float wa = wy[yo * 4 + a];
#pragma unroll
    for (int b = 0; b < 4; ++b) {
      float v[8];
      V8<T>::ld(x + cb8_index(n, cb, ys, ix[xo * 4 + b], C8, Hi, Wi), v);
      if (act >= 0) {
        act_fwd8<FastMath<T>::value>(v, sc, sh, act, v);
#pragma unroll
        for (int j = 0; j < 8; ++j) v[j] = round_storage<T>(v[j]);
      }
      float w = wa * wx[xo * 4 + b];
#pragma unroll
      for (int j = 0; j < 8; ++j) acc[j] += w * v[j];
    }
  }
}

template <typename T> struct XformRaw;
template <> struct XformRaw<bf16_t> {
  static __device__ __forceinline__ void apply(uint4 (&r)[1], const float (&sc)[8], const float (&sh)[8], int act) {
    r[0] = xform_bf16x8(r[0], sc, sh, act);
  }
};
template <> struct XformRaw<f16_t> {
  static __device__ __forceinline__ void apply(uint4 (&r)[1], const float (&sc)[8], const float (&sh)[8], int act) {
    r[0] = xform_f16x8(r[0], sc, sh, act);
  }
};
template <> struct XformRaw<float> {
// ... 967 lines not shown
  else if (dtype == MC_BF16) {
    switch (gkind_of(s0, s1)) { case 1: APP(bf16_t, 1); break; case 2: APP(bf16_t, 2); break; case 3: APP(bf16_t, 3); break; default: APP(bf16_t, 0); }
  } else if (dtype == MC_MIX16) {
    switch (gkind_of(s0, s1)) { case 1: APPH(1); break; case 2: APPH(2); break; case 3: APPH(3); break; default: APPH(0); }
  } else return MC_EUNSUPPORTED;
#undef APPH
#undef APP
  MC_CHECK_LAUNCH();
  return MC_OK;
}

int mc_gn_act_fwd_small(const void* y, const float* stat_partials, int32_t tiles, int32_t n, int32_t c, int32_t h, int32_t w,
                        int32_t groups, float eps, const float* gamma, const float* beta, int32_t act, int32_t pool,
                        int32_t dtype, float* stats_out, void* a_out, void* pooled, void* stream) {
  GnArgs a;
  int rc = fill_gn_args(a, n, c, h, w, groups, stats_out, gamma, beta, MC_POST_GN_ACT, act);
  if (rc) return rc;
  if (!y || !stat_partials || tiles <= 0 || !gamma || !beta || !stats_out || !a_out || (pool > 1 && !pooled)) return MC_EINVAL;
  if (pool != 1 && pool != 2) return MC_EUNSUPPORTED;
  if (a.cpg != 1 && a.cpg != 2 && a.cpg != 4 && a.cpg != 8) return MC_EUNSUPPORTED;
  dim3 g(a.C8, n);
  hipStream_t s = (hipStream_t)stream;
#define FS(T, P) hipLaunchKernelGGL((k_gn_act_small<T, P>), g, dim3(gn_small_threads(a.C8 * n)), 0, s, a, (const T*)y, stat_partials, tiles, eps, stats_out, (T*)a_out, (T*)pooled)
  if (dtype == MC_F32) { if (pool == 1) FS(float, 1); else FS(float, 2); }
  else if (dtype == MC_BF16) { if (pool == 1) FS(bf16_t, 1); else FS(bf16_t, 2); }
  else if (dtype == MC_MIX16) { if (pool == 1) FS(f16_t, 1); else FS(f16_t, 2); }
  else return MC_EUNSUPPORTED;
#undef FS
  MC_CHECK_LAUNCH();
  return MC_OK;
}

int mc_gn_act_bwd_small(const void* y, int32_t n, int32_t c, int32_t h, int32_t w, int32_t groups, const float* stats,
                        const float* gamma, const float* beta, int32_t act, int32_t dtype, const mc_grad_src* g0,
                        const mc_grad_src* g1, void* dy, float* chan_sums, void* stream) {
  GnArgs a;
  int rc = fill_gn_args(a, n, c, h, w, groups, stats, gamma, beta, MC_POST_GN_ACT, act);
  if (rc) return rc;
  if (!y || !dy || !g0 || !stats || !gamma || !beta || !chan_sums) return MC_EINVAL;
  if (a.cpg != 1 && a.cpg != 2 && a.cpg != 4 && a.cpg != 8) return MC_EUNSUPPORTED;
  if ((rc = check_gsrc(g0)) || (rc = check_gsrc(g1))) return rc;
  dim3 g(a.C8, n);
  hipStream_t s = (hipStream_t)stream;
  const mc_grad_src s0 = gsrc_or_none(g0), s1 = gsrc_or_none(g1);
  const int CP = a.C8 * 8;
#define SM(T, GK) hipLaunchKernelGGL((k_gn_bwd_small<T, GK>), g, dim3(gn_small_threads(a.C8 * n)), 0, s, a, (const T*)y, s0, s1, (T*)dy, chan_sums, CP)
#define SMH(GK) hipLaunchKernelGGL((k_gn_bwd_small<bf16_t, GK, f16_t>), g, dim3(gn_small_threads(a.C8 * n)), 0, s, a, (const f16_t*)y, s0, s1, (bf16_t*)dy, chan_sums, CP)
  if (dtype == MC_F32) SM(float, 0);
  else if (dtype == MC_BF16) {
    switch (gkind_of(s0, s1)) { case 1: SM(bf16_t, 1); break; case 2: SM(bf16_t, 2); break; case 3: SM(bf16_t, 3); break; default: SM(bf16_t, 0); }
  } else if (dtype == MC_MIX16) {
    switch (gkind_of(s0, s1)) { case 1: SMH(1); break; case 2: SMH(2); break; case 3: SMH(3); break; default: SMH(0); }
  } else return MC_EUNSUPPORTED;
#undef SMH
#undef SM
  MC_CHECK_LAUNCH();
  return MC_OK;
}

int mc_gn_param_grads_batched(const float* const* chan_sums, const int32_t* n, const int32_t* c, float* const* dgamma,
                              float* const* dbeta, int32_t jobs, void* stream) {
  if (!chan_sums || !n || !c || !dgamma || !dbeta || jobs <= 0) return MC_EINVAL;
  for (int base = 0; base < jobs; base += GP_MAX) {
    GpTable t;
    t.n = jobs - base < GP_MAX ? jobs - base : GP_MAX;
    int first = 0;
    for (int k = 0; k < t.n; ++k) {
      const int i = base + k;
      if (!chan_sums[i] || n[i] <= 0 || c[i] <= 0) return MC_EINVAL;
      t.j[k].pc = chan_sums[i]; t.j[k].dgamma = dgamma[i]; t.j[k].dbeta = dbeta[i];
      t.j[k].N = n[i]; t.j[k].C = c[i]; t.j[k].CP = ((c[i] + 7) / 8) * 8; t.j[k].first = first;
      first += ((c[i] + 63) / 64) * 64;
    }
    hipLaunchKernelGGL(k_gn_param_grads, dim3(first / 64), dim3(64), 0, (hipStream_t)stream, t);
  }
  MC_CHECK_LAUNCH();
  return MC_OK;
}

int mc_fold_padded2(void* buf0, int32_t c0, void* buf1, int32_t c1, int32_t n, int32_t hs, int32_t ws, int32_t pad, int32_t pad_mode,
                    int32_t dtype, void* stream) {
  if (!buf0 || n <= 0 || c0 <= 0 || hs <= 0 || ws <= 0 || pad < 0 || pad > 2 || (buf1 && c1 <= 0)) return MC_EINVAL;
  if (pad == 0 || pad_mode == MC_PAD_ZEROS) return MC_OK;
  const int C8a = (c0 + 7) / 8, C8 = C8a + (buf1 ? (c1 + 7) / 8 : 0), t = pad + 1;
  int all = (hs < 2 * t || ws < 2 * t) ? 1 : 0;
  int total = all ? hs * ws : 2 * t * ws + (hs - 2 * t) * 2 * t;
  dim3 g(cdiv(total, 256), C8, n);
  hipStream_t s = (hipStream_t)stream;
  if (dtype == MC_F32) hipLaunchKernelGGL(k_fold_padded<float>, g, dim3(256), 0, s, (float*)buf0, C8, hs, ws, pad, pad_mode, all, (float*)buf1, C8a);
  else if (mc_is16(dtype)) hipLaunchKernelGGL(k_fold_padded<bf16_t>, g, dim3(256), 0, s, (bf16_t*)buf0, C8, hs, ws, pad, pad_mode, all, (bf16_t*)buf1, C8a);
  else return MC_EUNSUPPORTED;
  MC_CHECK_LAUNCH();
  return MC_OK;
}

int mc_fold_padded(void* buf, int32_t n, int32_t c, int32_t hs, int32_t ws, int32_t pad, int32_t pad_mode, int32_t dtype,
                   void* stream) {
  if (!buf || c <= 0) return MC_EINVAL;
  return mc_fold_padded2(buf, c, nullptr, 0, n, hs, ws, pad, pad_mode, dtype, stream);
}

static void fold_shape(int hs, int ws, int pad, int& all, int& total) {
  const int t = pad + 1;
  all = (hs < 2 * t || ws < 2 * t) ? 1 : 0;
  total = all ? hs * ws : 2 * t * ws + (hs - 2 * t) * 2 * t;
}

int32_t mc_fold_blocks(int32_t hs, int32_t ws, int32_t pad, int32_t pad_mode) {
  if (hs <= 0 || ws <= 0 || pad <= 0 || pad_mode == MC_PAD_ZEROS) return 0;
  int all, total;
  fold_shape(hs, ws, pad, all, total);
  return cdiv(total, 256);
}

int mc_fold_padded_dz(void* buf, int32_t n, int32_t c, int32_t hs, int32_t ws, int32_t pad, int32_t pad_mode, int32_t dtype,
                      const void* y, const float* coef, int32_t act, float* partials, int32_t part_stride_blocks,
                      int32_t part_first_block, void* stream) {
  if (!buf || !y || !partials || n <= 0 || c <= 0 || hs <= 0 || ws <= 0 || pad < 0 || pad > 2) return MC_EINVAL;
  if (act < MC_ACT_NONE || act > MC_ACT_ELU) return MC_EINVAL;
  const int blocks = mc_fold_blocks(hs, ws, pad, pad_mode);
  if (blocks == 0) return MC_OK;
  if (part_first_block < 0 || part_first_block + blocks > part_stride_blocks) return MC_EINVAL;
  int all, total;
  fold_shape(hs, ws, pad, all, total);
  const int C8 = (c + 7) / 8;
  dim3 g(blocks, C8, n);
  hipStream_t s = (hipStream_t)stream;
  if (dtype == MC_F32) hipLaunchKernelGGL(k_fold_padded_dz<float>, g, dim3(256), 0, s, (float*)buf, C8, hs, ws, pad, pad_mode, all, (const float*)y, coef, act, partials, part_stride_blocks, part_first_block);
  else if (dtype == MC_BF16) hipLaunchKernelGGL(k_fold_padded_dz<bf16_t>, g, dim3(256), 0, s, (bf16_t*)buf, C8, hs, ws, pad, pad_mode, all, (const bf16_t*)y, coef, act, partials, part_stride_blocks, part_first_block);
  else if (dtype == MC_MIX16) hipLaunchKernelGGL((k_fold_padded_dz<bf16_t, f16_t>), g, dim3(256), 0, s, (bf16_t*)buf, C8, hs, ws, pad, pad_mode, all, (const f16_t*)y, coef, act, partials, part_stride_blocks, part_first_block);
  else return MC_EUNSUPPORTED;
  MC_CHECK_LAUNCH();
  return MC_OK;
}

int mc_gn_bwd_apply_dz(const mc_grad_src* dz, const void* y, int32_t n, int32_t c, int32_t h, int32_t w, int32_t groups,
                       const float* coef, const float* m12, int32_t dtype, void* dy, void* stream) {
  if (!dz || !dy || n <= 0 || c <= 0 || h <= 0 || w <= 0) return MC_EINVAL;
  if (coef && (!y || !m12 || groups <= 0 || c % groups != 0)) return MC_EINVAL;
  int rc = check_gsrc(dz);
  if (rc) return rc;
  if ((dz->kind != MC_GSRC_PADFOLD && dz->kind != MC_GSRC_PLAIN) || dz->c8_total != 0 || dz->hs != h || dz->ws != w) return MC_EUNSUPPORTED;
  const int rows = gn_apply_rows(h, w), C8 = (c + 7) / 8;
  dim3 g(cdiv(h, rows), C8, n);
  hipStream_t s = (hipStream_t)stream;
  const int gr = groups > 0 ? groups : 1;
#define APZ(T, GK) hipLaunchKernelGGL((k_gn_bwd_apply_dz<T, GK>), g, dim3(256), 0, s, *dz, (const T*)y, c, C8, h, w, gr, coef, m12, (T*)dy, rows)
  if (dtype == MC_F32) { if (dz->kind == MC_GSRC_PADFOLD) APZ(float, MC_GSRC_PADFOLD); else APZ(float, MC_GSRC_PLAIN); }
  else if (dtype == MC_BF16) { if (dz->kind == MC_GSRC_PADFOLD) APZ(bf16_t, MC_GSRC_PADFOLD); else APZ(bf16_t, MC_GSRC_PLAIN); }
  else if (dtype == MC_MIX16) {
#define APZH(GK) hipLaunchKernelGGL((k_gn_bwd_apply_dz<bf16_t, GK, f16_t>), g, dim3(256), 0, s, *dz, (const f16_t*)y, c, C8, h, w, gr, coef, m12, (bf16_t*)dy, rows)
    if (dz->kind == MC_GSRC_PADFOLD) APZH(MC_GSRC_PADFOLD); else APZH(MC_GSRC_PLAIN);
#undef APZH
  }
  else return MC_EUNSUPPORTED;
#undef APZ
  MC_CHECK_LAUNCH();
  return MC_OK;
}

int mc_rect_copy(const void* src, int32_t hs, int32_t ws, int32_t sy, int32_t sx, void* dst, int32_t hd, int32_t wd,
                 int32_t dy, int32_t dx, int32_t rh, int32_t rw, int32_t n, int32_t c, int32_t accumulate, int32_t dtype,
                 void* stream) {
  if (!dst || n <= 0 || c <= 0 || rh <= 0 || rw <= 0) return MC_EINVAL;
  if (dy < 0 || dx < 0 || dy + rh > hd || dx + rw > wd) return MC_EINVAL;
  if (src && (sy < 0 || sx < 0 || sy + rh > hs || sx + rw > ws)) return MC_EINVAL;
  const int C8 = (c + 7) / 8;
  dim3 g(max(1, min(cdiv(rh * rw, 256), 512)), C8, n);
  hipStream_t s = (hipStream_t)stream;
  if (dtype == MC_F32) hipLaunchKernelGGL(k_rect_copy<float>, g, dim3(256), 0, s, (const float*)src, hs, ws, sy, sx, (float*)dst, hd, wd, dy, dx, rh, rw, C8, accumulate);
  else if (dtype == MC_MIX16) hipLaunchKernelGGL(k_rect_copy<f16_t>, g, dim3(256), 0, s, (const f16_t*)src, hs, ws, sy, sx, (f16_t*)dst, hd, wd, dy, dx, rh, rw, C8, accumulate);
  else if (dtype == MC_BF16) hipLaunchKernelGGL(k_rect_copy<bf16_t>, g, dim3(256), 0, s, (const bf16_t*)src, hs, ws, sy, sx, (bf16_t*)dst, hd, wd, dy, dx, rh, rw, C8, accumulate);
  else return MC_EUNSUPPORTED;
  MC_CHECK_LAUNCH();
  return MC_OK;
}

int mc_concat_cb8(const void* const* srcs, const int32_t* src_c, int32_t n_src, int32_t n, int32_t h, int32_t w,
                  int32_t dtype, void* out, void* stream) {
  if (!srcs || !src_c || !out || n_src < 1 || n_src > CAT_MAX || n <= 0 || h <= 0 || w <= 0) return MC_EINVAL;
  bool aligned = true;
  for (int k = 0; k < n_src; ++k) {
    if (!srcs[k] || src_c[k] <= 0) return MC_EINVAL;
    if (k < n_src - 1 && (src_c[k] % 8) != 0) aligned = false;
  }
  if (dtype != MC_F32 && !mc_is16(dtype)) return MC_EUNSUPPORTED;
  hipStream_t s = (hipStream_t)stream;
  if (!aligned) {
// ... 239 lines not shown
```

### pbml_mantle_convection_amd/engine.py

```python
from __future__ import annotations

import ctypes as C
import os
from dataclasses import dataclass, field
from typing import Dict, List, Optional, Tuple

import numpy as np
import torch

from . import _lib as L

DTYPES = {"fp32": (L.MC_F32, torch.float32), "f32": (L.MC_F32, torch.float32),
          "bf16": (L.MC_BF16, torch.bfloat16), "mixed": (L.MC_MIX16, torch.float16)}


@dataclass
class ConvNode:
    name: str
    srcs: List[int]
    out: int
    c_out: int
    k: int
    pad: int
    sym_h: int
# ... 310 lines not shown
                for name, r in regs.items()})
        else:
            ho, wo = h + 2 * node.pad - k + 1, w + 2 * node.pad - k + 1
            final_f32 = node.post == L.POST_NONE and node is g.nodes[-1] and mc != L.MC_F32 and node.c_out <= 16
            convs[i] = ConvShape(dgrad, *_conv_descs(N, h, w, cs, node.c_out, k, node.pad, mode, mc, mcg,
                                                     (node.sym_h, node.sym_v, node.sym_hv), final_f32, dgrad), final_f32)
        size[node.out] = (ho, wo)
        grad[node.out] = True
        if node.pool > 1:
            size[node.pooled] = (ho // node.pool, wo // node.pool)
            grad[node.pooled] = True
    return size, grad, convs


def iter_conv_descs(g: NetGraph, N: int, H: int, W: int, precision: str):
    for i, c in shape_walk(g, N, H, W, precision)[2].items():
        if c.banks is None:
            yield g.nodes[i].name, c.d, c.dd
        else:
            for name, (_, d, dd) in c.banks.items():
                yield g.nodes[i].name + name, d, dd


def bicubic_tables(n_in: int, n_out: int):
    A = -0.75
    scale = n_in / n_out
    o = np.arange(n_out, dtype=np.float64)
    real = scale * (o + 0.5) - 0.5
    i0 = np.floor(real)
    t = real - i0

    def c1(x):
        return ((A + 2) * x - (A + 3)) * x * x + 1

    def c2(x):
        return ((A * x - 5 * A) * x + 8 * A) * x - 4 * A
    w = np.stack([c2(t + 1), c1(t), c1(1 - t), c2(2 - t)], 1)
    idx = np.clip(i0[:, None] + np.arange(-1, 3)[None, :], 0, n_in - 1).astype(np.int32)
    lists = [dict() for _ in range(n_in)]
    for oo in range(n_out):
        for k in range(4):
            d = lists[idx[oo, k]]
            d[oo] = d.get(oo, 0.0) + w[oo, k]
    start = np.zeros(n_in + 1, np.int32)
    tj, tw = [], []
    for i in range(n_in):
        for oo in sorted(lists[i]):
            tj.append(oo)
            tw.append(lists[i][oo])
        start[i + 1] = len(tj)
    return (idx, w.astype(np.float32), start, np.asarray(tj, np.int32), np.asarray(tw, np.float32))


@dataclass
class _T:
    C: int
    H: int = 0
    W: int = 0
    buf: Optional[torch.Tensor] = None
    requires_grad: bool = True
    gsrcs: list = field(default_factory=list)
    fused: bool = False
    raw: Optional[torch.Tensor] = None
    coef: Optional[torch.Tensor] = None
    act: int = 0


class Engine:

    def __init__(self, graph: NetGraph, precision: str = "fp32"):
        if precision not in DTYPES:
            raise ValueError(f"precision must be one of {list(DTYPES)}")
        L.load()
        self.g = graph
        self.precision = "fp32" if precision == "f32" else precision
        self.mc_dtype, self.t_dtype = DTYPES[precision]
        self.mc_gdtype, self.g_dtype = (L.MC_BF16, torch.bfloat16) if self.mc_dtype == L.MC_MIX16 else (self.mc_dtype, self.t_dtype)
        self.shape = None
        self._tables = {}
        self.fuse = int(os.environ.get("MANTLE_FUSE", "0"))
        self.fuse_maxpix = int(os.environ.get("MANTLE_FUSE_MAXPIX", str(128 * 128)))
        self.fuse_dz_rr = precision == "mixed" and os.environ.get("MANTLE_FUSE_DZ_RR", "1") != "0"
        self.gn_small_pix = int(os.environ.get("MANTLE_GN_SMALL_PIX", str(64 * 64 + 4)))

    def freeze(self):
        self._frozen = True

    def configure(self, N: int, H: int, W: int, device):
        if self.shape == (N, H, W, str(device)):
            return
        if getattr(self, "_frozen", False):
            raise RuntimeError(f"this engine is pinned to input shape {self.shape[:3]} by a captured HIP graph; got {(N, H, W)} "
                               "(use a separate module / engine instance, or an un-captured trainer, for another shape)")
        g = self.g
        if H % g.divisor or W % g.divisor:
            raise ValueError(f"input H, W must be divisible by {g.divisor}")
        self.device = device
        self.N = N
        size, grad, convs = shape_walk(g, N, H, W, self.precision)
        T: Dict[int, _T] = {tid: _T(C=c, H=size[tid][0], W=size[tid][1], requires_grad=grad[tid])
                            for tid, c in g.channels.items()}
        self.mode = L.PAD_MODES[g.pad_mode]
        f32 = dict(dtype=torch.float32, device=device)
        self.plan = []
        max_dy = 0

        def cb8(c, h, w):
            return torch.empty((N, (c + 7) // 8, h, w, 8), dtype=self.t_dtype, device=device)

        def cb8g(c, h, w):
            return torch.empty((N, (c + 7) // 8, h, w, 8), dtype=self.g_dtype, device=device)

        T[0].buf = cb8(T[0].C, T[0].H, T[0].W)
        cons: Dict[int, list] = {tid: [] for tid in g.channels}
        for node in g.nodes:
            for i in (node.srcs if node.kind in ("conv", "cat") else [node.src]):
                cons[i].append(node)
        self.cons = cons
        self.prod = {}
        for i, node in enumerate(g.nodes):
            if node.kind == "up":
                s, o = T[node.src], T[node.out]
                o.buf = cb8(o.C, o.H, o.W)
                tabs = (self._table(s.H, o.H), self._table(s.W, o.W))
                e = dict(node=node, tabs=tabs, dsrc=cb8g(s.C, s.H, s.W),
                         maxtaps=tuple(int(np.diff(bicubic_tables(a, b)[2]).max()) for a, b in ((s.H, o.H), (s.W, o.W))))
                if o.H > 3 * s.H or o.W > 3 * s.W:
                    e["bws"] = torch.empty((N, (s.C + 7) // 8, s.H, o.W, 8), **f32)
                self.plan.append(e)
                continue
            if node.kind == "pool":
                o = T[node.out]
                o.buf = cb8(o.C, o.H, o.W)
                self.plan.append(dict(node=node, dsum=cb8g(o.C, o.H, o.W)))
                continue
            if node.kind == "cat":
                o = T[node.out]
                o.buf = cb8(o.C, o.H, o.W)
                gather, off = {}, 0
                for k, t in enumerate(node.srcs):
                    c = T[t].C
                    if T[t].requires_grad and (off % 8 or (k < len(node.srcs) - 1 and c % 8)):
                        gather[t] = (off, cb8g(c, o.H, o.W))
                    off += c
                self.plan.append(dict(node=node, gather=gather))
                continue
            o = T[node.out]
            plan = self._plan_learned if node.learned else self._plan_conv
            e = plan(node, convs[i], [T[t] for t in node.srcs], o, cb8, cb8g, f32)
            if node.pool > 1:
                T[node.pooled].buf = cb8(node.c_out, T[node.pooled].H, T[node.pooled].W)
            max_dy = max(max_dy, N * e["coutp"] * o.H * o.W)
            self.plan.append(e)
        self.T = T
        self.dY = torch.empty(max_dy, dtype=self.g_dtype, device=device)
        self.convs = [e for e in self.plan if e["node"].kind == "conv" and not e["node"].learned]
        self.learned = [e for e in self.plan if e["node"].kind == "conv" and e["node"].learned]
        self.lws = torch.empty(max([e["lws_bytes"] for e in self.learned] + [0]), dtype=torch.uint8, device=device)
        last = self.plan[-1]
        assert last["node"].kind == "conv", "graph must end in a conv node"
        self.final_plain = last["node"].post == L.POST_NONE
        assert self.final_plain or not g.subtract_mean
        fo = T[last["node"].out]
        self.out_h, self.out_w = fo.H, fo.W - 2 * g.crop_w
        self.dOut = None if self.final_plain else cb8g(fo.C, fo.H, fo.W)
        self.chan_mean = torch.empty((N, g.c_out), **f32) if g.subtract_mean else None
# ... 299 lines not shown
                continue
            if node.kind == "pool":
                s, o = T[node.src], T[node.out]
                assert 1 <= len(o.gsrcs) <= 2
                if not s.requires_grad:
                    continue
                q = o.gsrcs[0]
                if len(o.gsrcs) == 1 and q.kind == L.GSRC_PADFOLD and q.c8_total == 0:
                    s.gsrcs.append(L.GradSrc(q.ptr, L.GSRC_PADFOLD_POOL, q.pad, q.pad_mode, node.f, o.H, o.W))
                else:
                    g1 = C.byref(o.gsrcs[1]) if len(o.gsrcs) > 1 else None
                    L.call("mc_gsrc_sum", C.byref(q), g1, N, o.C, o.H, o.W, self.mc_gdtype, L.ptr(e["dsum"]), st)
                    s.gsrcs.append(L.GradSrc(L.ptr(e["dsum"]), L.GSRC_PLAIN_POOL, 0, 0, node.f, o.H, o.W))
                continue
            if node.kind == "up":
                s, o = T[node.src], T[node.out]
                assert len(o.gsrcs) == 1, "an upsampled tensor feeds exactly one conv"
                (iy, wy, tys, tyj, tyw), (_, _, txs, txj, txw) = e["tabs"]
                if "bws" not in e and e["maxtaps"][1] <= 12:
                    L.call("mc_bicubic_bwd_walk", C.byref(o.gsrcs[0]), N, s.C, s.H, s.W, o.H, o.W, L.ptr(iy), L.ptr(wy), L.ptr(tys),
                           L.ptr(tyj), L.ptr(txs), L.ptr(txj), L.ptr(txw), e["maxtaps"][1], self.mc_gdtype, L.ptr(e["dsrc"]), st)
                elif "bws" in e:
                    L.call("mc_bicubic_bwd_separable", C.byref(o.gsrcs[0]), N, s.C, s.H, s.W, o.H, o.W, L.ptr(tys), L.ptr(tyj),
                           L.ptr(tyw), L.ptr(txs), L.ptr(txj), L.ptr(txw), self.mc_gdtype, L.ptr(e["bws"]), L.ptr(e["dsrc"]), st)
                else:
                    L.call("mc_bicubic_bwd_taps", C.byref(o.gsrcs[0]), N, s.C, s.H, s.W, o.H, o.W, L.ptr(tys), L.ptr(tyj),
                           L.ptr(tyw), L.ptr(txs), L.ptr(txj), L.ptr(txw), e["maxtaps"][0], e["maxtaps"][1], self.mc_gdtype,
                           L.ptr(e["dsrc"]), st)
                s.gsrcs.append(L.GradSrc(L.ptr(e["dsrc"]), L.GSRC_PLAIN, 0, 0, 1, s.H, s.W))
                continue
            d = e["desc"]
            o = T[node.out]
            srcs = [T[i] for i in node.srcs]
            if node.post != L.POST_NONE and "dz" in e:
                assert not o.gsrcs, f"{node.name}: fused dz and separate gradient sources"
                if node.post == L.POST_GN_ACT:
                    gamma = self._param(params, node.gn_name + "weight")
                    if "dz_pc" in e:
                        L.call("mc_gn_act_bwd_finalize_n", L.ptr(e["dz_part"]), N, e["dz_blocks"], node.c_out, node.groups,
                               o.H * o.W, L.ptr(gamma), L.ptr(e["m12"]), L.ptr(e["dz_pc"]), st)
                        gp_jobs.append((L.ptr(e["dz_pc"]), node.c_out, L.ptr(grads[node.gn_name + "weight"]),
                                        L.ptr(grads[node.gn_name + "bias"])))
                    else:
                        L.call("mc_gn_act_bwd_finalize", L.ptr(e["dz_part"]), N, e["dz_blocks"], node.c_out, node.groups,
                               o.H * o.W, L.ptr(gamma), L.ptr(e["m12"]), L.ptr(grads[node.gn_name + "weight"]),
                               L.ptr(grads[node.gn_name + "bias"]), st)
                L.call("mc_gn_bwd_apply_dz", C.byref(e["dz"]), L.ptr(e["Y"]), N, node.c_out, o.H, o.W, max(node.groups, 1),
                       L.ptr(e["coef"]) if node.post == L.POST_GN_ACT else None, L.ptr(e.get("m12")), self.mc_dtype,
                       L.ptr(dY), st)
                del e["dz"]
            elif node.post != L.POST_NONE:
                gs = list(o.gsrcs)
                if node.pool > 1:
                    p = T[node.pooled]
                    for q in p.gsrcs:
                        assert q.kind in (L.GSRC_PADFOLD, L.GSRC_PLAIN) and q.c8_total == 0, "a pooled tensor feeds exactly one conv"
                        kind = L.GSRC_PADFOLD_POOL if q.kind == L.GSRC_PADFOLD else L.GSRC_PLAIN_POOL
                        gs.append(L.GradSrc(q.ptr, kind, q.pad, q.pad_mode, node.pool, p.H, p.W))
                assert 1 <= len(gs) <= 2, f"{node.name}: {len(gs)} gradient sources"
                g0 = C.byref(gs[0])
                g1 = C.byref(gs[1]) if len(gs) > 1 else None
                gamma = self._param(params, node.gn_name + "weight") if node.gn_name else None
                beta = self._param(params, node.gn_name + "bias") if node.gn_name else None
                if node.post == L.POST_GN_ACT and "pc" in e:
                    L.call("mc_gn_act_bwd_small", L.ptr(e["Y"]), N, node.c_out, o.H, o.W, node.groups, L.ptr(e["stats"]),
                           L.ptr(gamma), L.ptr(beta), act, self.mc_dtype, g0, g1, L.ptr(dY), L.ptr(e["pc"]), st)
                    gp_jobs.append((L.ptr(e["pc"]), node.c_out, L.ptr(grads[node.gn_name + "weight"]),
                                    L.ptr(grads[node.gn_name + "bias"])))
                else:
                    if node.post == L.POST_GN_ACT:
                        L.call("mc_gn_act_bwd_reduce", L.ptr(e["Y"]), N, node.c_out, o.H, o.W, node.groups,
                               L.ptr(e["stats"]), L.ptr(gamma), L.ptr(beta), node.post, act, self.mc_dtype, g0, g1,
                               L.ptr(e["gpart"]), st)
                        L.call("mc_gn_act_bwd_finalize", L.ptr(e["gpart"]), N, e["gblocks"], node.c_out, node.groups,
                               o.H * o.W, L.ptr(gamma), L.ptr(e["m12"]), L.ptr(grads[node.gn_name + "weight"]),
                               L.ptr(grads[node.gn_name + "bias"]), st)
                    L.call("mc_gn_act_bwd_apply", L.ptr(e["Y"]), N, node.c_out, o.H, o.W, node.groups,
                           L.ptr(e.get("stats")), L.ptr(e.get("m12")), L.ptr(gamma), L.ptr(beta), node.post, act,
                           self.mc_dtype, g0, g1, L.ptr(dY), st)
            if node.learned:
                self._learned_backward(e, srcs[0], dY, params, grads, st)
                continue
            x0, x1, pro = self._sources(srcs)
            L.call("mc_conv2d_wgrad_fused", C.byref(d), x0, x1, pro, L.ptr(dY), L.ptr(e["wpart"]), st)
            if e["need_dgrad"]:
                dxp = e["dxp"]
                pe = e.get("epi")
                if pe is not None:
                    pn, s0 = pe["node"], srcs[0]
                    coef = L.ptr(pe["coef"]) if pn.post == L.POST_GN_ACT else None
                    epi = L.ConvEpilogue(L.ptr(pe["Y"]), coef, act, node.pad, self.mode, s0.H, s0.W, L.ptr(pe["dz_part"]),
                                         pe["dz_blocks"], int(self.mc_dtype == L.MC_MIX16))
                    self._probe_begin()
                    L.call("mc_conv2d_fused", C.byref(e["ddesc"]), L.ptr(dY), None, None, L.ptr(e["dbank"]), None,
                           L.ptr(dxp[0]), None, None, C.byref(epi), st)
                    self._probe_end(e["ddesc"], "dgrad+dz " + node.name, extra_in=s0.C * s0.H * s0.W)
                    L.call("mc_fold_padded_dz", L.ptr(dxp[0]), N, s0.C, s0.H, s0.W, node.pad, self.mode, self.mc_dtype,
                           L.ptr(pe["Y"]), coef, act, L.ptr(pe["dz_part"]), pe["dz_blocks"], pe["dz_tiles"], st)
                    pe["dz"] = L.GradSrc(L.ptr(dxp[0]), L.GSRC_PADFOLD, node.pad, self.mode, 1, s0.H, s0.W)
                    continue
                self._probe_begin()
                L.call("mc_conv2d", C.byref(e["ddesc"]), L.ptr(dY), None, L.ptr(e["dbank"]), None, L.ptr(dxp[0]),
                       L.ptr(dxp[1]) if len(dxp) > 1 else None, None, st)
                self._probe_end(e["ddesc"], "dgrad " + node.name)
                live = [(s, buf) for s, buf in zip(srcs, dxp) if s.requires_grad]
                if len(live) == 2 and (live[0][0].H, live[0][0].W) == (live[1][0].H, live[1][0].W):
                    L.call("mc_fold_padded2", L.ptr(live[0][1]), live[0][0].C, L.ptr(live[1][1]), live[1][0].C, N, live[0][0].H,
                           live[0][0].W, node.pad, self.mode, self.mc_gdtype, st)
                else:
                    for s, buf in live:
                        L.call("mc_fold_padded", L.ptr(buf), N, s.C, s.H, s.W, node.pad, self.mode, self.mc_gdtype, st)
                for s, buf in live:
                    s.gsrcs.append(L.GradSrc(L.ptr(buf), L.GSRC_PADFOLD, node.pad, self.mode, 1, s.H, s.W))
        if gp_jobs:
            n = len(gp_jobs)
            L.call("mc_gn_param_grads_batched", (C.c_void_p * n)(*[j[0] for j in gp_jobs]), (C.c_int32 * n)(*([N] * n)),
                   (C.c_int32 * n)(*[j[1] for j in gp_jobs]), (C.c_void_p * n)(*[j[2] for j in gp_jobs]),
                   (C.c_void_p * n)(*[j[3] for j in gp_jobs]), n, st)
        jobs = [(e["desc"], e["wpart"], e["node"].name + "weight", e["node"].name + "bias") for e in self.convs]
        jobs += [(e["desc"], e["wpart"], e["node"].name + "conv.weight", e["node"].name + "learnable_bias") for e in self.learned]
        n = len(jobs)
        if n:
            descs = (L.ConvDesc * n)(*[j[0] for j in jobs])
            parts = (C.c_void_p * n)(*[L.ptr(j[1]) for j in jobs])
            dws = (C.c_void_p * n)(*[L.ptr(grads[j[2]]) for j in jobs])
            dbs = (C.c_void_p * n)(*[L.ptr(grads[j[3]]) for j in jobs])
            L.call("mc_conv2d_wgrad_finalize_batched", descs, parts, dws, dbs, n, st)

    def _pack_all_banks(self, params, st):
        jobs = []
        for e in self.convs:
            w = self._param(params, e["node"].name + "weight")
            jobs.append((e["desc"], L.ptr(w), 0, L.ptr(e["bank"])))
            if e["need_dgrad"]:
                jobs.append((e["desc"], L.ptr(w), 1, L.ptr(e["dbank"])))
        for e in self.learned:
            w = self._param(params, e["node"].name + "conv.weight")
            jobs.append((e["fdesc"], L.ptr(w), 0, L.ptr(e["bank"])))
            if e["need_dgrad"]:
                jobs.append((e["desc"], L.ptr(w), 1, L.ptr(e["dbank"])))
        n = len(jobs)
        if n:
            descs = (L.ConvDesc * n)(*[j[0] for j in jobs])
            ws = (C.c_void_p * n)(*[j[1] for j in jobs])
            dg = (C.c_int32 * n)(*[j[2] for j in jobs])
            outs = (C.c_void_p * n)(*[j[3] for j in jobs])
            L.call("mc_pack_weights_batched", descs, ws, dg, outs, n, st)
        n = len(self.learned)
        if n:
            descs = (L.LearnedDesc * n)(*[e["ldesc"] for e in self.learned])
            ws = (C.c_void_p * (8 * n))(*[L.ptr(self._param(params, e["node"].name + b + ".weight"))
                                          for e in self.learned for b in L.LEARNED_FRAME_BANKS])
            fw = (C.c_void_p * n)(*[L.ptr(e["lbank"]) for e in self.learned])
            dg = (C.c_void_p * n)(*[L.ptr(e["ldbank"]) for e in self.learned])
            L.call("mc_learned_pack_banks_batched", descs, ws, fw, dg, n, st)

    _probe = None

    def enable_probe(self, passes: int = 3):
        self._probe = []
        n = 2 * (2 * len(getattr(self, "convs", [])) + 8) * max(passes, 1)
        self._probe_pool = [torch.cuda.Event(enable_timing=True) for _ in range(n)]
        for ev in self._probe_pool:
            ev.record()
        torch.cuda.synchronize()
        return self._probe

    def disable_probe(self):
        self._probe = None
        self._probe_pool = []

    def _probe_event(self):
        ev = self._probe_pool.pop() if getattr(self, "_probe_pool", None) else torch.cuda.Event(enable_timing=True)
        ev.record()
        return ev

    def _probe_begin(self):
        if self._probe is not None:
            self._probe_ev = self._probe_event()

    def _probe_end(self, d, label, extra_in=0):
        if self._probe is not None:
            ev = self._probe_event()
            es = torch.tensor([], dtype=self.t_dtype).element_size()
            ho, wo = d.h + 2 * d.pad - d.k + 1, d.w + 2 * d.pad - d.k + 1
            cin = d.c_in0 + d.c_in1
            nbytes = d.n * es * (cin * d.h * d.w + d.c_out * ho * wo + extra_in)
            flops = 2.0 * d.n * cin * d.c_out * d.k * d.k * ho * wo
            name = L.load().mc_conv_kernel_name(C.byref(d)).decode()
            shape = f"{label.split()[0]} {cin}->{d.c_out} k{d.k} {d.n}x{d.h}x{d.w}"
            self._probe.append((name, shape, self._probe_ev, ev, nbytes, flops))

    @staticmethod
    def kernel_family(name):
        return name.split(",")[0].rstrip(">") + ">"

# ... 59 lines not shown
```

Before: 3236 samples/s.

## Fold padded-gradient reflection pass into the wgrad kernel launch

Moves the padded-gradient fold (plain or dz variant) so it runs inside the bf16 wgrad MFMA kernel: each block first does a grid-strided share of fold work, then its normal weight-gradient tile. The wgrad launch is moved after dgrad so the fold can piggyback on it, which removes one separate kernel launch per padded conv layer in backward. The cost is extra work and shared-memory use at the start of the wgrad blocks, which may delay the wgrad compute and adds complexity. Non-bf16 or prologue-fused paths fall back to a separate fold call.

```diff
diff --git a/include/mantle_hip.h b/include/mantle_hip.h
--- a/include/mantle_hip.h
+++ b/include/mantle_hip.h
@@ -101,6 +101,18 @@
                              float* dbias, void* stream);
 int mc_conv2d_wgrad_fused(const mc_conv_desc* d, const void* x0, const void* x1, const mc_conv_prologue* pro,
                           const void* dy, void* partials, void* stream);
+typedef struct {
+  void* buf0; int32_t c0;
+  void* buf1; int32_t c1;
+  int32_t n, hs, ws, pad, pad_mode, dtype;
+  const void* y;
+  const float* coef;
+  int32_t act;
+  float* partials;
+  int32_t part_stride_blocks, part_first_block;
+} mc_wgrad_fold;
+int mc_conv2d_wgrad_fold(const mc_conv_desc* d, const void* x0, const void* x1, const mc_conv_prologue* pro,
+                         const void* dy, void* partials, const mc_wgrad_fold* fold, void* stream);
 int mc_pack_weights_batched(const mc_conv_desc* descs, const float* const* w_unique, const int32_t* dgrad,
                             void* const* packed, int32_t n, void* stream);
 int mc_conv2d_wgrad_finalize_batched(const mc_conv_desc* descs, const void* const* partials, float* const* dw_unique,
diff --git a/pbml_mantle_convection_amd/_lib.py b/pbml_mantle_convection_amd/_lib.py
--- a/pbml_mantle_convection_amd/_lib.py
+++ b/pbml_mantle_convection_amd/_lib.py
@@ -43,6 +43,13 @@
                 ("y_f16", C.c_int32)]
 
 
+class WgradFold(C.Structure):
+    _fields_ = [("buf0", C.c_void_p), ("c0", C.c_int32), ("buf1", C.c_void_p), ("c1", C.c_int32), ("n", C.c_int32),
+                ("hs", C.c_int32), ("ws", C.c_int32), ("pad", C.c_int32), ("pad_mode", C.c_int32), ("dtype", C.c_int32),
+                ("y", C.c_void_p), ("coef", C.c_void_p), ("act", C.c_int32), ("partials", C.c_void_p),
+                ("part_stride_blocks", C.c_int32), ("part_first_block", C.c_int32)]
+
+
 class LossDesc(C.Structure):
     _fields_ = [("n", C.c_int32), ("h", C.c_int32), ("w", C.c_int32), ("p_pred", C.c_int32),
                 ("loss_type", C.c_int32), ("loss_scale", C.c_int32), ("loss_derivative", C.c_int32),
@@ -54,6 +61,7 @@
 _CD, _GS, _LD = C.POINTER(ConvDesc), C.POINTER(GradSrc), C.POINTER(LossDesc)
 _CP, _CE = C.POINTER(ConvPrologue), C.POINTER(ConvEpilogue)
 _LN = C.POINTER(LearnedDesc)
+_WF = C.POINTER(WgradFold)
 
 SIGNATURES = {
     "mc_version": (C.c_int, []),
@@ -70,6 +78,7 @@
     "mc_conv2d": (C.c_int, [_CD, _vp, _vp, _vp, _vp, _vp, _vp, _vp, _vp]),
     "mc_conv2d_fused": (C.c_int, [_CD, _vp, _vp, _CP, _vp, _vp, _vp, _vp, _vp, _CE, _vp]),
     "mc_conv2d_wgrad_fused": (C.c_int, [_CD, _vp, _vp, _CP, _vp, _vp, _vp]),
+    "mc_conv2d_wgrad_fold": (C.c_int, [_CD, _vp, _vp, _CP, _vp, _vp, _WF, _vp]),
     "mc_gn_finalize_coef": (C.c_int, [_vp, _i32, _i32, _i32, _i32, _i32, _f32, _vp, _vp, _vp, _vp, _vp]),
     "mc_fold_blocks": (_i32, [_i32, _i32, _i32, _i32]),
     "mc_fold_padded_dz": (C.c_int, [_vp, _i32, _i32, _i32, _i32, _i32, _i32, _i32, _vp, _vp, _i32, _vp, _i32, _i32, _vp]),
diff --git a/pbml_mantle_convection_amd/build_ext.py b/pbml_mantle_convection_amd/build_ext.py
--- a/pbml_mantle_convection_amd/build_ext.py
+++ b/pbml_mantle_convection_amd/build_ext.py
@@ -6,7 +6,7 @@
 CSRC = os.path.join(HERE, "csrc")
 LIB = os.path.join(HERE, "libmantle_hip.so")
 SOURCES = ["elementwise.hip", "conv_api.hip", "conv_f32.hip", "conv_bf16.hip", "conv_rr_bf16.hip", "conv_learned.hip", "loss.hip", "optim.hip"]
-HEADERS = ["common.h", "conv_common.h", "conv_rr.h", os.path.join("..", "..", "include", "mantle_hip.h")]
+HEADERS = ["common.h", "conv_common.h", "conv_rr.h", "fold_padded.h", os.path.join("..", "..", "include", "mantle_hip.h")]
 FLAGS = ["-O3", "--offload-arch=gfx950", "-fPIC", "-std=c++17", "-Wall", "-Wno-unused-function",
          "-ffp-contract=off"]
 
diff --git a/pbml_mantle_convection_amd/csrc/common.h b/pbml_mantle_convection_amd/csrc/common.h
--- a/pbml_mantle_convection_amd/csrc/common.h
+++ b/pbml_mantle_convection_amd/csrc/common.h
@@ -283,20 +283,6 @@
   return w;
 }
 
-__device__ __forceinline__ int fold_candidates(int i, int n, int p, int mode, int (&out)[6]) {
-  int cnt = 0;
-  out[cnt++] = i + p;
-  if (mode == MC_PAD_REFLECT) {
-    if (i >= 1 && i <= p) out[cnt++] = p - i;
-    int j = 2 * (n - 1) - i;
-    if (j >= n && j < n + p) out[cnt++] = j + p;
-  } else if (mode == MC_PAD_REPLICATE) {
-    if (i == 0) for (int q = 0; q < p && cnt < 6; ++q) out[cnt++] = q;
-    if (i == n - 1) for (int q = 0; q < p && cnt < 6; ++q) out[cnt++] = n + p + q;
-  }
-  return cnt;
-}
-
 template <typename T, int KIND = -1>
 __device__ __forceinline__ void grad_fetch_add(const mc_grad_src& g, int n, int cb, int y, int x, int C8,
                                                float (&acc)[8]) {
diff --git a/pbml_mantle_convection_amd/csrc/conv_api.hip b/pbml_mantle_convection_amd/csrc/conv_api.hip
--- a/pbml_mantle_convection_amd/csrc/conv_api.hip
+++ b/pbml_mantle_convection_amd/csrc/conv_api.hip
@@ -1,4 +1,5 @@
 #include "conv_rr.h"
+#include "fold_padded.h"
 
 int mc_conv2d_f32(const ConvGeom& g, const void* x0, const void* x1, const void* bank, const float* bias, void* y0,
                   void* y1, float* part, const ConvFuse& fz, int fuse, hipStream_t s);
@@ -9,7 +10,7 @@
 int mc_conv2d_bf16(const ConvGeom& g, const void* x0, const void* x1, const void* bank, const float* bias, void* y0,
                    void* y1, float* part, const ConvFuse& fz, int fuse, hipStream_t s);
 int mc_wgrad_bf16(const ConvGeom& g, const void* x0, const void* x1, const void* dy, void* part, const ConvFuse& fz, int fuse,
-                  hipStream_t s);
+                  const FoldJob& fj, hipStream_t s);
 const char* mc_bf16_kernel_name(const ConvGeom& g);
 void mc_bf16_bank_dims(const ConvGeom& g, int dgrad, int& chunks, int& steps, int& ntiles);
 bool mc_rr_applies(int dtype, int cout, int wo, bool full_pad);
@@ -281,8 +282,27 @@
   return (size_t)g.wgrad_G * wg_slab_floats(g.CoutP, g.CinP, g.K * g.K) * sizeof(float);
 }
 
-int mc_conv2d_wgrad_fused(const mc_conv_desc* d, const void* x0, const void* x1, const mc_conv_prologue* pro,
-                          const void* dy, void* partials, void* stream) {
+static int fold_job_for(const mc_wgrad_fold* f, int conv_dtype, FoldJob& j) {
+  j = fold_job_none();
+  if (!f->buf0 || f->n <= 0 || f->c0 <= 0 || f->hs <= 0 || f->ws <= 0 || f->pad < 0 || f->pad > 2) return MC_EINVAL;
+  const bool dz = f->y != nullptr;
+  if (dz ? (f->buf1 != nullptr || !f->partials || f->act < MC_ACT_NONE || f->act > MC_ACT_ELU) : (f->buf1 && f->c1 <= 0)) return MC_EINVAL;
+  if (dz ? f->dtype != conv_dtype : !mc_is16(f->dtype)) return MC_EUNSUPPORTED;
+  const int blocks = mc_fold_blocks(f->hs, f->ws, f->pad, f->pad_mode);
+  if (blocks == 0) return MC_OK;
+  if (dz && (f->part_first_block < 0 || f->part_first_block + blocks > f->part_stride_blocks)) return MC_EINVAL;
+  int total;
+  fold_shape(f->hs, f->ws, f->pad, j.all, total);
+  j.buf = f->buf0; j.buf1 = f->buf1; j.y = f->y; j.coef = f->coef; j.part = f->partials;
+  j.C8a = (f->c0 + 7) / 8; j.C8 = j.C8a + (f->buf1 ? (f->c1 + 7) / 8 : 0);
+  j.H = f->hs; j.W = f->ws; j.p = f->pad; j.mode = f->pad_mode; j.act = f->act;
+  j.stride = f->part_stride_blocks; j.first = f->part_first_block;
+  j.gx = blocks; j.gy = j.C8; j.gz = f->n;
+  return MC_OK;
+}
+
+int mc_conv2d_wgrad_fold(const mc_conv_desc* d, const void* x0, const void* x1, const mc_conv_prologue* pro,
+                         const void* dy, void* partials, const mc_wgrad_fold* fold, void* stream) {
   ConvGeom g;
   int rc = geom_for(d, g);
   if (rc) return rc;
@@ -290,8 +310,25 @@
   ConvFuse fz = conv_fuse_none();
   const int fuse = fill_prologue(pro, fz, rc);
   if (rc) return rc;
-  if (mc_is16(g.dtype)) return mc_wgrad_bf16(g, x0, x1, dy, partials, fz, fuse, (hipStream_t)stream);
+  if (mc_is16(g.dtype) && !fuse) {
+    FoldJob fj = fold_job_none();
+    if (fold && (rc = fold_job_for(fold, g.dtype, fj))) return rc;
+    return mc_wgrad_bf16(g, x0, x1, dy, partials, fz, fuse, fj, (hipStream_t)stream);
+  }
+  if (fold) {
+    const mc_wgrad_fold& f = *fold;
+    rc = f.y ? mc_fold_padded_dz(f.buf0, f.n, f.c0, f.hs, f.ws, f.pad, f.pad_mode, f.dtype, f.y, f.coef, f.act, f.partials,
+                                 f.part_stride_blocks, f.part_first_block, stream)
+             : mc_fold_padded2(f.buf0, f.c0, f.buf1, f.c1, f.n, f.hs, f.ws, f.pad, f.pad_mode, f.dtype, stream);
+    if (rc) return rc;
+  }
+  if (mc_is16(g.dtype)) return mc_wgrad_bf16(g, x0, x1, dy, partials, fz, fuse, fold_job_none(), (hipStream_t)stream);
   return mc_wgrad_f32(g, x0, x1, dy, partials, fz, fuse, (hipStream_t)stream);
+}
+
+int mc_conv2d_wgrad_fused(const mc_conv_desc* d, const void* x0, const void* x1, const mc_conv_prologue* pro,
+                          const void* dy, void* partials, void* stream) {
+  return mc_conv2d_wgrad_fold(d, x0, x1, pro, dy, partials, nullptr, stream);
 }
 
 int mc_conv2d_wgrad(const mc_conv_desc* d, const void* x0, const void* x1, const void* dy, void* partials,
diff --git a/pbml_mantle_convection_amd/csrc/conv_bf16.hip b/pbml_mantle_convection_amd/csrc/conv_bf16.hip
--- a/pbml_mantle_convection_amd/csrc/conv_bf16.hip
+++ b/pbml_mantle_convection_amd/csrc/conv_bf16.hip
@@ -1,4 +1,5 @@
 #include "conv_common.h"
+#include "fold_padded.h"
 #include <type_traits>
 
 using bf16x8 = __attribute__((ext_vector_type(8))) short;
@@ -408,7 +409,8 @@
 template <int K, int NTW, bool PRO = false, bool XH = false>
 __global__ __launch_bounds__(256, NTW == 1 ? 3 : 2) void k_wgrad_mfma_bf16(ConvGeom g, const bf16_t* __restrict__ x0,
                                                             const bf16_t* __restrict__ x1, const bf16_t* __restrict__ dy,
-                                                            float* __restrict__ part, int tiles_x, int tiles, ConvFuse fz) {
+                                                            float* __restrict__ part, int tiles_x, int tiles, ConvFuse fz,
+                                                            FoldJob fj) {
   constexpr int NS = 4;
   constexpr int TPW = (K * K + NS) / NS;
   constexpr int KK = K * K;
@@ -424,6 +426,11 @@
   constexpr int D_ELEMS = NTW * 2 * WTH * WTW, D_ITERS = D_ELEMS / 256;
   static_assert(D_ELEMS % 256 == 0, "dy tile must divide evenly over the threads");
   __shared__ uint4 smem[2 * XPS + NTW * 2 * DPS];
+  if constexpr (!PRO)
+  if (fj.gx)
+    fold_job_run<bf16_t, typename std::conditional<XH, f16_t, bf16_t>::type>(
+        fj, blockIdx.x + gridDim.x * (blockIdx.y + gridDim.y * blockIdx.z), gridDim.x * gridDim.y * gridDim.z,
+        reinterpret_cast<float*>(smem));
   uint4* const xs = smem;
   uint4* const ds = smem + 2 * XPS;
   const int chunk = blockIdx.y, cog = blockIdx.z;
@@ -740,7 +747,7 @@
 }
 
 int mc_wgrad_bf16(const ConvGeom& g_in, const void* x0, const void* x1, const void* dy, void* part, const ConvFuse& fz,
-                  int fuse, hipStream_t s) {
+                  int fuse, const FoldJob& fj, hipStream_t s) {
   const ConvGeom& g = g_in;
   const int tiles_x = (g.Wo + WTW - 1) / WTW, tiles_y = (g.Ho + WTH - 1) / WTH;
   const int tiles = tiles_x * tiles_y;
@@ -750,7 +757,7 @@
   const bool xh = g.dtype == MC_MIX16;
 #define WLAUNCH_X(K, NTW, PRO, XH)                                                                                     \
   hipLaunchKernelGGL((k_wgrad_mfma_bf16<K, NTW, PRO, XH>), grid, dim3(256), 0, s, g, (const bf16_t*)x0, (const bf16_t*)x1, \
-                     (const bf16_t*)dy, (float*)part, tiles_x, tiles, fz)
+                     (const bf16_t*)dy, (float*)part, tiles_x, tiles, fz, fj)
 #define WLAUNCH_P(K, NTW, PRO) do { if (xh) WLAUNCH_X(K, NTW, PRO, true); else WLAUNCH_X(K, NTW, PRO, false); } while (0)
 #define WLAUNCH(K, NTW) do { if (fuse) WLAUNCH_P(K, NTW, true); else WLAUNCH_P(K, NTW, false); } while (0)
   if (g.K == 5) { if (ntw == 1) WLAUNCH(5, 1); else WLAUNCH(5, 2); }
diff --git a/pbml_mantle_convection_amd/csrc/elementwise.hip b/pbml_mantle_convection_amd/csrc/elementwise.hip
--- a/pbml_mantle_convection_amd/csrc/elementwise.hip
+++ b/pbml_mantle_convection_amd/csrc/elementwise.hip
@@ -1,4 +1,5 @@
 #include "common.h"
+#include "fold_padded.h"
 
 namespace {
 
@@ -733,110 +734,16 @@
 
 template <typename T>
 __global__ void k_fold_padded(T* __restrict__ buf, int C8, int H, int W, int p, int mode, int all, T* __restrict__ buf1, int C8a) {
-  const int n = blockIdx.z;
-  int cb = blockIdx.y;
-  if (buf1 && cb >= C8a) { buf = buf1; cb -= C8a; C8 -= C8a; } else if (buf1) { C8 = C8a; }
-  const int t = p + 1;
-  const int band = all ? H * W : 2 * t * W;
-  const int side = all ? 0 : (H - 2 * t) * 2 * t;
-  const int Hp = H + 2 * p, Wp = W + 2 * p;
-  for (int i = blockIdx.x * blockDim.x + threadIdx.x; i < band + side; i += gridDim.x * blockDim.x) {
-    int yy, xx;
-    if (all) {
-      yy = i / W;
-      xx = i - yy * W;
-    } else if (i < band) {
-      int r = i / W;
-      xx = i - r * W;
-      yy = r < t ? r : H - 2 * t + r;
-    } else {
-      int k = i - band;
-      int r = k / (2 * t), c = k - r * 2 * t;
-      yy = t + r;
-      xx = c < t ? c : W - 2 * t + c;
-    }
-    int cy[6], cx[6];
-    int ny = fold_candidates(yy, H, p, mode, cy), nx = fold_candidates(xx, W, p, mode, cx);
-    if (ny == 1 && nx == 1) continue;
-    float acc[8] = {0, 0, 0, 0, 0, 0, 0, 0};
-    for (int a = 0; a < ny; ++a)
-      for (int b = 0; b < nx; ++b) {
-        float v[8];
-        V8<T>::ld(buf + cb8_index(n, cb, cy[a], cx[b], C8, Hp, Wp), v);
-#pragma unroll
-        for (int j = 0; j < 8; ++j) acc[j] += v[j];
-      }
-    V8<T>::st(buf + cb8_index(n, cb, yy + p, xx + p, C8, Hp, Wp), acc);
-  }
+  fold_padded_block<T>(buf, C8, H, W, p, mode, all, buf1, C8a, blockIdx.x, blockIdx.y, blockIdx.z, gridDim.x);
 }
 
 template <typename T, typename TY = T>
 __global__ __launch_bounds__(256) void k_fold_padded_dz(T* __restrict__ buf, int C8, int H, int W, int p, int mode, int all,
                                                         const TY* __restrict__ y, const float* __restrict__ coef4, int act,
                                                         float* __restrict__ part, int stride, int first) {
-  const int n = blockIdx.z, cb = blockIdx.y;
-  const int t = p + 1;
-  const int band = all ? H * W : 2 * t * W;
-  const int side = all ? 0 : (H - 2 * t) * 2 * t;
-  const int Hp = H + 2 * p, Wp = W + 2 * p, CP = C8 * 8;
-  float sc[8], sh[8], me[8], rs[8];
-#pragma unroll
-  for (int j = 0; j < 8; ++j) {
-    if (coef4) {
-      const float4 c4 = reinterpret_cast<const float4*>(coef4)[(size_t)n * CP + cb * 8 + j];
-      sc[j] = c4.x; sh[j] = c4.y; me[j] = c4.z; rs[j] = c4.w;
-    } else { sc[j] = 1.f; sh[j] = 0.f; me[j] = 0.f; rs[j] = 0.f; }
-  }
-  float s[16];
-#pragma unroll
-  for (int j = 0; j < 16; ++j) s[j] = 0.f;
-  const int i = blockIdx.x * blockDim.x + threadIdx.x;
-  if (i < band + side) {
-    int yy, xx;
-    if (all) {
-      yy = i / W;
-      xx = i - yy * W;
-    } else if (i < band) {
-      int r = i / W;
-      xx = i - r * W;
-      yy = r < t ? r : H - 2 * t + r;
-    } else {
-      int k = i - band;
-      int r = k / (2 * t), c = k - r * 2 * t;
-      yy = t + r;
-      xx = c < t ? c : W - 2 * t + c;
-    }
-    int cy[6], cx[6];
-    const int ny = fold_candidates(yy, H, p, mode, cy), nx = fold_candidates(xx, W, p, mode, cx);
-    float acc[8] = {0, 0, 0, 0, 0, 0, 0, 0};
-    for (int a = 0; a < ny; ++a)
-      for (int b = 0; b < nx; ++b) {
-        float v[8];
-        V8<T>::ld(buf + cb8_index(n, cb, cy[a], cx[b], C8, Hp, Wp), v);
-#pragma unroll
-        for (int j = 0; j < 8; ++j) acc[j] += v[j];
-      }
-    float yv[8], gz[8];
-    V8<TY>::ld(y + cb8_index(n, cb, yy, xx, C8, H, W), yv);
-    act_bwd8<FastMath<T>::value>(yv, sc, sh, act, gz);
-#pragma unroll
-    for (int j = 0; j < 8; ++j) {
-      const float dz = acc[j] * gz[j];
-      acc[j] = dz;
-      s[2 * j] = dz;
-      s[2 * j + 1] = dz * (yv[j] - me[j]) * rs[j];
-    }
-    V8<T>::st(buf + cb8_index(n, cb, yy + p, xx + p, C8, Hp, Wp), acc);
-  }
-  __shared__ float red[4][16];
-  int idx;
-  float r = wave_sum16(s, threadIdx.x & 63, idx);
-  if ((threadIdx.x & 3) == 0) red[threadIdx.x >> 6][idx] = r;
-  __syncthreads();
-  if (threadIdx.x < 16) {
-    float tot = red[0][threadIdx.x] + red[1][threadIdx.x] + red[2][threadIdx.x] + red[3][threadIdx.x];
-    part[(((size_t)n * stride + first + blockIdx.x) * CP + cb * 8 + (threadIdx.x >> 1)) * 2 + (threadIdx.x & 1)] = tot;
-  }
+  __shared__ float red[64];
+  fold_padded_dz_block<T, TY>(buf, C8, H, W, p, mode, all, y, coef4, act, part, stride, first, blockIdx.x, blockIdx.y, blockIdx.z,
+                              red);
 }
 
 template <typename T, int GK, typename TY = T>
@@ -1970,9 +1877,9 @@
                     int32_t dtype, void* stream) {
   if (!buf0 || n <= 0 || c0 <= 0 || hs <= 0 || ws <= 0 || pad < 0 || pad > 2 || (buf1 && c1 <= 0)) return MC_EINVAL;
   if (pad == 0 || pad_mode == MC_PAD_ZEROS) return MC_OK;
-  const int C8a = (c0 + 7) / 8, C8 = C8a + (buf1 ? (c1 + 7) / 8 : 0), t = pad + 1;
-  int all = (hs < 2 * t || ws < 2 * t) ? 1 : 0;
-  int total = all ? hs * ws : 2 * t * ws + (hs - 2 * t) * 2 * t;
+  const int C8a = (c0 + 7) / 8, C8 = C8a + (buf1 ? (c1 + 7) / 8 : 0);
+  int all, total;
+  fold_shape(hs, ws, pad, all, total);
   dim3 g(cdiv(total, 256), C8, n);
   hipStream_t s = (hipStream_t)stream;
   if (dtype == MC_F32) hipLaunchKernelGGL(k_fold_padded<float>, g, dim3(256), 0, s, (float*)buf0, C8, hs, ws, pad, pad_mode, all, (float*)buf1, C8a);
@@ -1986,12 +1893,6 @@
                    void* stream) {
   if (!buf || c <= 0) return MC_EINVAL;
   return mc_fold_padded2(buf, c, nullptr, 0, n, hs, ws, pad, pad_mode, dtype, stream);
-}
-
-static void fold_shape(int hs, int ws, int pad, int& all, int& total) {
-  const int t = pad + 1;
-  all = (hs < 2 * t || ws < 2 * t) ? 1 : 0;
-  total = all ? hs * ws : 2 * t * ws + (hs - 2 * t) * 2 * t;
 }
 
 int32_t mc_fold_blocks(int32_t hs, int32_t ws, int32_t pad, int32_t pad_mode) {
diff --git a/pbml_mantle_convection_amd/csrc/fold_padded.h b/pbml_mantle_convection_amd/csrc/fold_padded.h
--- /dev/null
+++ b/pbml_mantle_convection_amd/csrc/fold_padded.h
@@ -0,0 +1,158 @@
+#pragma once
+#include "common.h"
+
+__device__ __forceinline__ int fold_count(int i, int n, int p, int mode) {
+  if (mode == MC_PAD_REFLECT) {
+    const int j = 2 * (n - 1) - i;
+    return 1 + ((i >= 1 && i <= p) ? 1 : 0) + ((j >= n && j < n + p) ? 1 : 0);
+  }
+  if (mode == MC_PAD_REPLICATE) return 1 + (i == 0 ? p : 0) + (i == n - 1 ? p : 0);
+  return 1;
+}
+__device__ __forceinline__ int fold_candidate(int i, int n, int p, int mode, int k) {
+  if (k == 0) return i + p;
+  if (mode == MC_PAD_REFLECT) {
+    if (k == 1 && i >= 1 && i <= p) return p - i;
+    return 2 * (n - 1) - i + p;
+  }
+  const int lo = i == 0 ? p : 0;
+  return k - 1 < lo ? k - 1 : n + p + (k - 1 - lo);
+}
+
+__device__ __forceinline__ void fold_frame_pixel(int i, int H, int W, int t, int band, int all, int& yy, int& xx) {
+  if (all) {
+    yy = i / W;
+    xx = i - yy * W;
+  } else if (i < band) {
+    int r = i / W;
+    xx = i - r * W;
+    yy = r < t ? r : H - 2 * t + r;
+  } else {
+    int k = i - band;
+    int r = k / (2 * t), c = k - r * 2 * t;
+    yy = t + r;
+    xx = c < t ? c : W - 2 * t + c;
+  }
+}
+
+template <typename T>
+__device__ __forceinline__ void fold_padded_block(T* __restrict__ buf, int C8, int H, int W, int p, int mode, int all,
+                                                  T* __restrict__ buf1, int C8a, int bx, int by, int bz, int gx) {
+  const int n = bz;
+  int cb = by;
+  if (buf1 && cb >= C8a) { buf = buf1; cb -= C8a; C8 -= C8a; } else if (buf1) { C8 = C8a; }
+  const int t = p + 1;
+  const int band = all ? H * W : 2 * t * W;
+  const int side = all ? 0 : (H - 2 * t) * 2 * t;
+  const int Hp = H + 2 * p, Wp = W + 2 * p;
+  for (int i = bx * 256 + threadIdx.x; i < band + side; i += gx * 256) {
+    int yy, xx;
+    fold_frame_pixel(i, H, W, t, band, all, yy, xx);
+    const int ny = fold_count(yy, H, p, mode), nx = fold_count(xx, W, p, mode);
+    if (ny == 1 && nx == 1) continue;
+    float acc[8] = {0, 0, 0, 0, 0, 0, 0, 0};
+    for (int a = 0; a < ny; ++a) {
+      const int cy = fold_candidate(yy, H, p, mode, a);
+      for (int b = 0; b < nx; ++b) {
+        float v[8];
+        V8<T>::ld(buf + cb8_index(n, cb, cy, fold_candidate(xx, W, p, mode, b), C8, Hp, Wp), v);
+#pragma unroll
+        for (int j = 0; j < 8; ++j) acc[j] += v[j];
+      }
+    }
+    V8<T>::st(buf + cb8_index(n, cb, yy + p, xx + p, C8, Hp, Wp), acc);
+  }
+}
+
+template <typename T, typename TY>
+__device__ __forceinline__ void fold_padded_dz_block(T* __restrict__ buf, int C8, int H, int W, int p, int mode, int all,
+                                                     const TY* __restrict__ y, const float* __restrict__ coef4, int act,
+                                                     float* __restrict__ part, int stride, int first, int bx, int by,
+                                                     int bz, float* red) {
+  const int n = bz, cb = by;
+  const int t = p + 1;
+  const int band = all ? H * W : 2 * t * W;
+  const int side = all ? 0 : (H - 2 * t) * 2 * t;
+  const int Hp = H + 2 * p, Wp = W + 2 * p, CP = C8 * 8;
+  float sc[8], sh[8], me[8], rs[8];
+#pragma unroll
+  for (int j = 0; j < 8; ++j) {
+    if (coef4) {
+      const float4 c4 = reinterpret_cast<const float4*>(coef4)[(size_t)n * CP + cb * 8 + j];
+      sc[j] = c4.x; sh[j] = c4.y; me[j] = c4.z; rs[j] = c4.w;
+    } else { sc[j] = 1.f; sh[j] = 0.f; me[j] = 0.f; rs[j] = 0.f; }
+  }
+  float s[16];
+#pragma unroll
+  for (int j = 0; j < 16; ++j) s[j] = 0.f;
+  const int i = bx * 256 + threadIdx.x;
+  if (i < band + side) {
+    int yy, xx;
+    fold_frame_pixel(i, H, W, t, band, all, yy, xx);
+    const int ny = fold_count(yy, H, p, mode), nx = fold_count(xx, W, p, mode);
+    float acc[8] = {0, 0, 0, 0, 0, 0, 0, 0};
+    for (int a = 0; a < ny; ++a) {
+      const int cy = fold_candidate(yy, H, p, mode, a);
+      for (int b = 0; b < nx; ++b) {
+        float v[8];
+        V8<T>::ld(buf + cb8_index(n, cb, cy, fold_candidate(xx, W, p, mode, b), C8, Hp, Wp), v);
+#pragma unroll
+        for (int j = 0; j < 8; ++j) acc[j] += v[j];
+      }
+    }
+    float yv[8], gz[8];
+    V8<TY>::ld(y + cb8_index(n, cb, yy, xx, C8, H, W), yv);
+    act_bwd8<FastMath<T>::value>(yv, sc, sh, act, gz);
+#pragma unroll
+    for (int j = 0; j < 8; ++j) {
+      const float dz = acc[j] * gz[j];
+      acc[j] = dz;
+      s[2 * j] = dz;
+      s[2 * j + 1] = dz * (yv[j] - me[j]) * rs[j];
+    }
+    V8<T>::st(buf + cb8_index(n, cb, yy + p, xx + p, C8, Hp, Wp), acc);
+  }
+  int idx;
+  float r = wave_sum16(s, threadIdx.x & 63, idx);
+  if ((threadIdx.x & 3) == 0) red[(threadIdx.x >> 6) * 16 + idx] = r;
+  __syncthreads();
+  if (threadIdx.x < 16) {
+    float tot = red[threadIdx.x] + red[16 + threadIdx.x] + red[32 + threadIdx.x] + red[48 + threadIdx.x];
+    part[(((size_t)n * stride + first + bx) * CP + cb * 8 + (threadIdx.x >> 1)) * 2 + (threadIdx.x & 1)] = tot;
+  }
+}
+
+struct FoldJob {
+  void* buf; void* buf1; const void* y; const float* coef; float* part;
+  int C8, C8a, H, W, p, mode, all, act, stride, first;
+  int gx, gy, gz;
+};
+static inline FoldJob fold_job_none() {
+  FoldJob j;
+  j.buf = j.buf1 = nullptr; j.y = nullptr; j.coef = nullptr; j.part = nullptr;
+  j.C8 = j.C8a = j.H = j.W = j.p = j.mode = j.all = j.act = j.stride = j.first = 0;
+  j.gx = j.gy = j.gz = 0;
+  return j;
+}
+
+static inline void fold_shape(int hs, int ws, int pad, int& all, int& total) {
+  const int t = pad + 1;
+  all = (hs < 2 * t || ws < 2 * t) ? 1 : 0;
+  total = all ? hs * ws : 2 * t * ws + (hs - 2 * t) * 2 * t;
+}
+
+template <typename T, typename TY>
+__device__ __forceinline__ void fold_job_run(const FoldJob& j, int block, int nb, float* red) {
+  const int total = j.gx * j.gy * j.gz;
+  for (int v = block; v < total; v += nb) {
+    const int bx = v % j.gx, r = v / j.gx;
+    const int by = r % j.gy, bz = r / j.gy;
+    if (j.y) {
+      fold_padded_dz_block<T, TY>((T*)j.buf, j.C8, j.H, j.W, j.p, j.mode, j.all, (const TY*)j.y, j.coef, j.act, j.part, j.stride,
+                                  j.first, bx, by, bz, red);
+      __syncthreads();
+    } else {
+      fold_padded_block<T>((T*)j.buf, j.C8, j.H, j.W, j.p, j.mode, j.all, (T*)j.buf1, j.C8a, bx, by, bz, j.gx);
+    }
+  }
+}
diff --git a/pbml_mantle_convection_amd/engine.py b/pbml_mantle_convection_amd/engine.py
--- a/pbml_mantle_convection_amd/engine.py
+++ b/pbml_mantle_convection_amd/engine.py
@@ -416,6 +416,7 @@
         self.fuse_maxpix = int(os.environ.get("MANTLE_FUSE_MAXPIX", str(128 * 128)))
         self.fuse_dz_rr = precision == "mixed" and os.environ.get("MANTLE_FUSE_DZ_RR", "1") != "0"
         self.gn_small_pix = int(os.environ.get("MANTLE_GN_SMALL_PIX", str(64 * 64 + 4)))
+        self.fold_in_wgrad = os.environ.get("MANTLE_FOLD_IN_WGRAD", "1") != "0"
 
     def freeze(self):
         self._frozen = True
@@ -881,7 +882,10 @@
                 self._learned_backward(e, srcs[0], dY, params, grads, st)
                 continue
             x0, x1, pro = self._sources(srcs)
-            L.call("mc_conv2d_wgrad_fused", C.byref(d), x0, x1, pro, L.ptr(dY), L.ptr(e["wpart"]), st)
+            ride = self.fold_in_wgrad and e["need_dgrad"] and node.pad > 0 and self.mode != L.PAD_MODES["zeros"]
+            if not ride:
+                L.call("mc_conv2d_wgrad_fused", C.byref(d), x0, x1, pro, L.ptr(dY), L.ptr(e["wpart"]), st)
+            fold = None
             if e["need_dgrad"]:
                 dxp = e["dxp"]
                 pe = e.get("epi")
@@ -894,23 +898,35 @@
                     L.call("mc_conv2d_fused", C.byref(e["ddesc"]), L.ptr(dY), None, None, L.ptr(e["dbank"]), None,
                            L.ptr(dxp[0]), None, None, C.byref(epi), st)
                     self._probe_end(e["ddesc"], "dgrad+dz " + node.name, extra_in=s0.C * s0.H * s0.W)
-                    L.call("mc_fold_padded_dz", L.ptr(dxp[0]), N, s0.C, s0.H, s0.W, node.pad, self.mode, self.mc_dtype,
-                           L.ptr(pe["Y"]), coef, act, L.ptr(pe["dz_part"]), pe["dz_blocks"], pe["dz_tiles"], st)
+                    if ride:
+                        fold = L.WgradFold(L.ptr(dxp[0]), s0.C, None, 0, N, s0.H, s0.W, node.pad, self.mode, self.mc_dtype,
+                                           L.ptr(pe["Y"]), coef, act, L.ptr(pe["dz_part"]), pe["dz_blocks"], pe["dz_tiles"])
+                    else:
+                        L.call("mc_fold_padded_dz", L.ptr(dxp[0]), N, s0.C, s0.H, s0.W, node.pad, self.mode, self.mc_dtype,
+                               L.ptr(pe["Y"]), coef, act, L.ptr(pe["dz_part"]), pe["dz_blocks"], pe["dz_tiles"], st)
                     pe["dz"] = L.GradSrc(L.ptr(dxp[0]), L.GSRC_PADFOLD, node.pad, self.mode, 1, s0.H, s0.W)
-                    continue
-                self._probe_begin()
-                L.call("mc_conv2d", C.byref(e["ddesc"]), L.ptr(dY), None, L.ptr(e["dbank"]), None, L.ptr(dxp[0]),
-                       L.ptr(dxp[1]) if len(dxp) > 1 else None, None, st)
-                self._probe_end(e["ddesc"], "dgrad " + node.name)
-                live = [(s, buf) for s, buf in zip(srcs, dxp) if s.requires_grad]
-                if len(live) == 2 and (live[0][0].H, live[0][0].W) == (live[1][0].H, live[1][0].W):
-                    L.call("mc_fold_padded2", L.ptr(live[0][1]), live[0][0].C, L.ptr(live[1][1]), live[1][0].C, N, live[0][0].H,
-                           live[0][0].W, node.pad, self.mode, self.mc_gdtype, st)
                 else:
+                    self._probe_begin()
+                    L.call("mc_conv2d", C.byref(e["ddesc"]), L.ptr(dY), None, L.ptr(e["dbank"]), None, L.ptr(dxp[0]),
+                           L.ptr(dxp[1]) if len(dxp) > 1 else None, None, st)
+                    self._probe_end(e["ddesc"], "dgrad " + node.name)
+                    live = [(s, buf) for s, buf in zip(srcs, dxp) if s.requires_grad]
+                    two = len(live) == 2 and (live[0][0].H, live[0][0].W) == (live[1][0].H, live[1][0].W)
+                    if ride and (two or len(live) == 1):
+                        s1, b1 = live[1] if two else (None, None)
+                        fold = L.WgradFold(L.ptr(live[0][1]), live[0][0].C, L.ptr(b1), s1.C if two else 0, N, live[0][0].H,
+                                           live[0][0].W, node.pad, self.mode, self.mc_gdtype, None, None, 0, None, 0, 0)
+                    elif two:
+                        L.call("mc_fold_padded2", L.ptr(live[0][1]), live[0][0].C, L.ptr(live[1][1]), live[1][0].C, N,
+                               live[0][0].H, live[0][0].W, node.pad, self.mode, self.mc_gdtype, st)
+                    else:
+                        for s, buf in live:
+                            L.call("mc_fold_padded", L.ptr(buf), N, s.C, s.H, s.W, node.pad, self.mode, self.mc_gdtype, st)
                     for s, buf in live:
-                        L.call("mc_fold_padded", L.ptr(buf), N, s.C, s.H, s.W, node.pad, self.mode, self.mc_gdtype, st)
-                for s, buf in live:
-                    s.gsrcs.append(L.GradSrc(L.ptr(buf), L.GSRC_PADFOLD, node.pad, self.mode, 1, s.H, s.W))
+                        s.gsrcs.append(L.GradSrc(L.ptr(buf), L.GSRC_PADFOLD, node.pad, self.mode, 1, s.H, s.W))
+            if ride:
+                L.call("mc_conv2d_wgrad_fold", C.byref(d), x0, x1, pro, L.ptr(dY), L.ptr(e["wpart"]),
+                       C.byref(fold) if fold is not None else None, st)
         if gp_jobs:
             n = len(gp_jobs)
             L.call("mc_gn_param_grads_batched", (C.c_void_p * n)(*[j[0] for j in gp_jobs]), (C.c_int32 * n)(*([N] * n)),
```

After: 3240 samples/s, median of 6. About the same (+0.1%).
